# sp-uhh/audio-visual-vad

Measured on AMD Instinct MI355X. Metric: AV frame-pairs/sec (fwd+bwd), higher is better.
Workload: dtype f32; 1 GPU; AV_net fused training step (WaveNet-W0 encoder + ResNet-18 trunk + concat + 2xLSTM1024 + FC, masked BCE, backward, RCCL all-reduce, fused Adam): BASELINE configs[3]/[4] per-GPU shard; per_gpu_frame_pairs=1024, global_frame_pairs=1024, sequences_per_gpu=64, parallelism=dp1, reserved_cus=0, reported_block=median

## Files before the change

audio-visual-vad_amd/csrc/wavenet.hip:

```cpp
#include "gemm_api.h"
#include "wn_block.h"
#include "wn_tail.h"

namespace {

static inline int grid1(long n) { long b = (n + 255) / 256; return (int)(b > 8192 ? 8192 : (b < 1 ? 1 : b)); }

__global__ void conv1d_fwd_generic(const float* __restrict__ x, const float* __restrict__ w, const float* __restrict__ bias,
                                   const float* __restrict__ res, float* __restrict__ y, int B, int Cin, int Cout, int Lin,
                                   int Lout, int fw, int dil, int relu_in, int res_off, int res_L) {
  const long n = (long)B * Cout * Lout;
  for (long i = (long)blockIdx.x * blockDim.x + threadIdx.x; i < n; i += (long)gridDim.x * blockDim.x) {
    const int t = (int)(i % Lout);
    const int co = (int)((i / Lout) % Cout);
    const int b = (int)(i / ((long)Lout * Cout));
    float acc = bias ? bias[co] : 0.f;
    const float* xb = x + (long)b * Cin * Lin + t;
    const float* wr = w + (long)co * Cin * fw;
    for (int ci = 0; ci < Cin; ++ci)
      for (int k = 0; k < fw; ++k) {
        float v = xb[(long)ci * Lin + k * dil];
        if (relu_in) v = fmaxf(v, 0.f);
        acc = fmaf(wr[ci * fw + k], v, acc);
      }
    if (res) acc += res[((long)b * Cout + co) * res_L + t + res_off];
    y[i] = acc;
  }
}

__global__ void conv1d_bwd_data_generic(const float* __restrict__ dy, const float* __restrict__ w,
                                        const float* __restrict__ xmask, const float* __restrict__ res, float* __restrict__ dx,
                                        int B, int Cin, int Cout, int Lin, int Lout, int fw, int dil, int res_off, int res_L) {
  const long n = (long)B * Cin * Lin;
  for (long i = (long)blockIdx.x * blockDim.x + threadIdx.x; i < n; i += (long)gridDim.x * blockDim.x) {
    const int ti = (int)(i % Lin);
    const int ci = (int)((i / Lin) % Cin);
    const int b = (int)(i / ((long)Lin * Cin));
    float acc = 0.f;
    if (!xmask || xmask[i] > 0.f) {
      for (int k = 0; k < fw; ++k) {
        const int to = ti - k * dil;
        if (to < 0 || to >= Lout) continue;
        const float* dyb = dy + (long)b * Cout * Lout + to;
        for (int co = 0; co < Cout; ++co) acc = fmaf(w[((long)co * Cin + ci) * fw + k], dyb[(long)co * Lout], acc);
      }
    }
    if (res && ti >= res_off && ti - res_off < res_L) acc += res[((long)b * Cin + ci) * res_L + ti - res_off];
    dx[i] = acc;
  }
}

__global__ void __launch_bounds__(256) chan_sum_acc(const float* __restrict__ dy, float* __restrict__ db, int B, int C, int L) {
  __shared__ float sm[256];
  const int c = blockIdx.x;
  float s = 0.f;
  for (int b = blockIdx.y; b < B; b += gridDim.y) {
    const float* p = dy + ((long)b * C + c) * L;
    for (int t = threadIdx.x; t < L; t += 256) s += p[t];
  }
  sm[threadIdx.x] = s;
  __syncthreads();
  for (int o = 128; o > 0; o >>= 1) {
    if (threadIdx.x < o) sm[threadIdx.x] += sm[threadIdx.x + o];
    __syncthreads();
  }
  if (threadIdx.x == 0) db[c] += sm[0];
}

__global__ void __launch_bounds__(256)
    narrow_conv1d_grads(const float* __restrict__ dy, const float* __restrict__ x, float* __restrict__ part,
                        int B, int Cout, int Cin, int Lout, int Lin, int fw) {
  __shared__ float sm[5][256];
  const int co = blockIdx.x, nw = Cin * fw;
  float acc[5] = {0.f, 0.f, 0.f, 0.f, 0.f};
  for (int b = blockIdx.y; b < B; b += gridDim.y) {
    const float* p = dy + ((long)b * Cout + co) * Lout;
    const float* xb = x + (long)b * Cin * Lin;
    for (int t = threadIdx.x; t < Lout; t += 256) {
      const float g = p[t];
      acc[4] += g;
#pragma unroll
      for (int j = 0; j < 4; ++j)
        if (j < nw) acc[j] = fmaf(g, xb[(long)(j / fw) * Lin + t + (j % fw)], acc[j]);
    }
  }
#pragma unroll
  for (int j = 0; j < 5; ++j) sm[j][threadIdx.x] = acc[j];
  __syncthreads();
  for (int o = 128; o > 0; o >>= 1) {
    if (threadIdx.x < o)
#pragma unroll
      for (int j = 0; j < 5; ++j) sm[j][threadIdx.x] += sm[j][threadIdx.x + o];
    __syncthreads();
  }
  if (threadIdx.x < 5) part[((long)blockIdx.y * Cout + co) * 5 + threadIdx.x] = sm[threadIdx.x][0];
}
__global__ void narrow_conv1d_grads_sum(const float* __restrict__ part, int ny, int Cout, int nw, float* __restrict__ dw,
                                        float* __restrict__ db) {
  const int i = blockIdx.x * blockDim.x + threadIdx.x;
  if (i >= Cout * 5) return;
  const int co = i / 5, j = i - co * 5;
  float s = 0.f;
  for (int y = 0; y < ny; ++y) s += part[((long)y * Cout + co) * 5 + j];
  if (j < 4) { if (j < nw && dw) dw[(long)co * nw + j] += s; }
  else if (db) db[co] += s;
}

template <int MODE>
__global__ void __launch_bounds__(256)
    wn_block_fwd_mfma(const float* __restrict__ s_in, const float* __restrict__ w_dil, const float* __restrict__ b_dil,
                      const float* __restrict__ w_dense, const float* __restrict__ b_dense, float* __restrict__ s_out,
                      float* __restrict__ z_out, int B, int Lin, int dil) {
  static_assert(MODE == 0 || MODE == 2, "s_out only, or z only");
  const int lane = threadIdx.x & 63;
  const int li = lane & 31, lh = lane >> 5;
  const int Lo = Lin - dil;
  const int tiles_per_seq = tiles_per_sequence<32>(Lo);
  const long ntiles = (long)B * tiles_per_seq;
  const long wave0 = ((long)blockIdx.x * blockDim.x + threadIdx.x) >> 6;
  const long nwaves = ((long)gridDim.x * blockDim.x) >> 6;

  __shared__ float wl[WIMG_SIZE];
  stage_block_weights(wl, w_dil, b_dil, w_dense, b_dense, threadIdx.x, 256);
  __syncthreads();
  float wd[32];
#pragma unroll
  for (int s = 0; s < 32; ++s) wd[s] = wl[WIMG_DIL + li * WIMG_DIL_PITCH + s * 2 + lh];
  float we[16];
#pragma unroll
  for (int r = 0; r < 16; ++r) we[r] = wl[WIMG_DENSE + li * WIMG_DENSE_PITCH + mfma32_row(r, lh)];
  const float* bzl = wl + WIMG_BDIL;
  const float* bsl = wl + WIMG_BDENSE;

  float xn[32], rn[16];
  auto issue = [&](long tile) {
    const TilePos p = tile_pos(tile < ntiles ? tile : ntiles - 1, tiles_per_seq, li, Lo);
    const int b = p.b, tcl = p.ok ? p.t : 0;
    const float* xp = s_in + (long)b * 32 * Lin + tcl + lh * dil;
#pragma unroll
    for (int c = 0; c < 32; ++c) xn[c] = xp[(long)c * Lin];
    if (MODE == 0) {
      const float* rp = s_in + (long)b * 32 * Lin + tcl + dil;
#pragma unroll
      for (int r = 0; r < 16; ++r) rn[r] = rp[(long)mfma32_row(r, lh) * Lin];
    }
  };
  if (wave0 < ntiles) issue(wave0);
  for (long tile = wave0; tile < ntiles; tile += nwaves) {
    const TilePos p = tile_pos(tile, tiles_per_seq, li, Lo);
    const int b = p.b, t = p.t;
    const bool ok = p.ok;
    float x[32], rv[16];
#pragma unroll
    for (int c = 0; c < 32; ++c) x[c] = ok ? xn[c] : 0.f;
#pragma unroll
    for (int r = 0; r < 16; ++r) rv[r] = (MODE == 0 && ok) ? rn[r] : 0.f;
    issue(tile + nwaves);
    f32x16 acc;
#pragma unroll
    for (int r = 0; r < 16; ++r) acc[r] = bzl[mfma32_row(r, lh)];
#pragma unroll
    for (int s = 0; s < 32; ++s) acc = mfma32(wd[s], relu1(x[s]), acc);
    if (MODE == 2) {
      float* zp = z_out + (long)b * 32 * Lo + t;
#pragma unroll
      for (int r = 0; r < 16; ++r)
        if (ok) zp[(long)mfma32_row(r, lh) * Lo] = acc[r];
    }
    if (MODE == 0) {
      f32x16 acc2;
#pragma unroll
      for (int r = 0; r < 16; ++r) acc2[r] = bsl[mfma32_row(r, lh)] + rv[r];
#pragma unroll
      for (int r = 0; r < 16; ++r) acc2 = mfma32(we[r], relu1(acc[r]), acc2);
      float* op = s_out + (long)b * 32 * Lo + t;
#pragma unroll
      for (int r = 0; r < 16; ++r)
        if (ok) op[(long)mfma32_row(r, lh) * Lo] = acc2[r];
    }
  }
}

struct FwdTile { float x[32], r[16]; };
template <bool RESIDENT>
__device__ __forceinline__ void wn_block_fwd_body(float* wl, const float* __restrict__ s_in, const float* __restrict__ w_dil,
                                                  const float* __restrict__ b_dil, const float* __restrict__ w_dense,
                                                  const float* __restrict__ b_dense, float* __restrict__ s_out, int B, int Lin,
                                                  int dil) {
  const int lane = threadIdx.x & 63;
  const int li = lane & 31, lh = lane >> 5;
  const int Lo = Lin - dil;
  const int tiles_per_seq = tiles_per_sequence<32>(Lo);
  const int ntiles = B * tiles_per_seq;
  const float* wdl = wl + WIMG_DIL + li * WIMG_DIL_PITCH + lh;
  const float* wel = wl + WIMG_DENSE + li * WIMG_DENSE_PITCH + 4 * lh;
  const float* bzl = wl + WIMG_BDIL + 4 * lh;
  const float* bsl = wl + WIMG_BDENSE + 4 * lh;
  const int rowL = Lin * 4, rowO = Lo * 4;
  float wd[32], we[16];

  auto issue = [&](int tile, FwdTile& n) __attribute__((always_inline)) {
    const TilePos p = tile_pos(RESIDENT && tile >= ntiles ? ntiles - 1 : tile, tiles_per_seq, li, Lo);
    const __amdgpu_buffer_rsrc_t rx = brsrc(s_in + (long)p.b * 32 * Lin, 32 * rowL);
    const int offx = p.ok ? (p.t + lh * dil) * 4 : BUF_OOB;
#pragma unroll
    for (int c = 0; c < 32; ++c) n.x[c] = bload(rx, offx, c * rowL);
    const int offr = p.ok ? (p.t + dil) * 4 + 4 * lh * rowL : BUF_OOB;
#pragma unroll
    for (int r = 0; r < 16; ++r) n.r[r] = bload(rx, offr, mfma32_row(r, 0) * rowL);
  };
  auto compute = [&](int tile, const FwdTile& c) __attribute__((always_inline)) {
    const TilePos p = tile_pos(tile, tiles_per_seq, li, Lo);
    const int offo = p.ok ? p.t * 4 + 4 * lh * rowO : BUF_OOB;
    f32x16 acc;
#pragma unroll
    for (int r = 0; r < 16; ++r) acc[r] = bzl[mfma32_row(r, 0)];
#pragma unroll
    for (int s = 0; s < 32; ++s) acc = mfma32(RESIDENT ? wd[s] : wdl[2 * s], relu1(c.x[s]), acc);
    f32x16 acc2;
#pragma unroll
    for (int r = 0; r < 16; ++r) acc2[r] = bsl[mfma32_row(r, 0)] + c.r[r];
#pragma unroll
    for (int r = 0; r < 16; ++r) acc2 = mfma32(RESIDENT ? we[r] : wel[mfma32_row(r, 0)], relu1(acc[r]), acc2);
    const __amdgpu_buffer_rsrc_t ro = brsrc(s_out + (long)p.b * 32 * Lo, 32 * rowO);
#pragma unroll
    for (int r = 0; r < 16; ++r) bstore(acc2[r], ro, offo, mfma32_row(r, 0) * rowO);
  };
  const TileWalkI w = xcd_walk_i(ntiles);
  FwdTile ta, tb;
  if (RESIDENT && w.first < w.last) issue(w.first, ta);
  stage_block_weights(wl, w_dil, b_dil, w_dense, b_dense, threadIdx.x, 256);
  __syncthreads();
  if (RESIDENT) {
#pragma unroll
    for (int s = 0; s < 32; ++s) wd[s] = wdl[2 * s];
#pragma unroll
    for (int r = 0; r < 16; ++r) we[r] = wel[mfma32_row(r, 0)];
    pingpong_tiles<false>(w, ta, tb, issue, compute);
  } else {
    plain_tiles<false, FwdTile>(w, issue, compute);
  }
}

__global__ void __launch_bounds__(256)
    wn_block_fwd_buf(const float* __restrict__ s_in, const float* __restrict__ w_dil, const float* __restrict__ b_dil,
                     const float* __restrict__ w_dense, const float* __restrict__ b_dense, float* __restrict__ s_out, int B,
                     int Lin, int dil) {
  __shared__ float wl[WIMG_SIZE];
  wn_block_fwd_body<true>(wl, s_in, w_dil, b_dil, w_dense, b_dense, s_out, B, Lin, dil);
}

__global__ void __launch_bounds__(256, 4)
    wn_block_fwd_occ(const float* __restrict__ s_in, const float* __restrict__ w_dil, const float* __restrict__ b_dil,
                     const float* __restrict__ w_dense, const float* __restrict__ b_dense, float* __restrict__ s_out, int B,
                     int Lin, int dil) {
  __shared__ float wl[WIMG_SIZE];
  wn_block_fwd_body<false>(wl, s_in, w_dil, b_dil, w_dense, b_dense, s_out, B, Lin, dil);
}

__global__ void __launch_bounds__(512, 4)
    wn_block_fwd_dma(const float* __restrict__ s_in, const float* __restrict__ w_dil, const float* __restrict__ b_dil,
                     const float* __restrict__ w_dense, const float* __restrict__ b_dense, float* __restrict__ s_out, int B, int Lin,
                     int dil) {
  const int lane = threadIdx.x & 63, wave = threadIdx.x >> 6;
  const int li = lane & 31, lh = lane >> 5;
  const int Lo = Lin - dil;
  const int tiles_per_seq = tiles_per_sequence<32>(Lo);
  const int ntiles = B * tiles_per_seq;
  __shared__ __attribute__((aligned(16))) float wl[8 * 2048 + WIMG_SIZE];
  float* const wts = wl + 8 * 2048;
  stage_block_weights(wts, w_dil, b_dil, w_dense, b_dense, threadIdx.x, 512);
  __syncthreads();
  const float* wdl = wts + WIMG_DIL + li * WIMG_DIL_PITCH + lh;
  const float* wel = wts + WIMG_DENSE + li * WIMG_DENSE_PITCH + 4 * lh;
  const float* bzl = wts + WIMG_BDIL + 4 * lh;
  const float* bsl = wts + WIMG_BDENSE + 4 * lh;
  const int rowL = Lin * 4, rowO = Lo * 4;
  float* const tb = wl + __builtin_amdgcn_readfirstlane(wave) * 2048;
  const float* const xs = tb + lh * 1024 + li;
  const float* const rs = tb + 1024 + 4 * lh * 32 + li;
  const int dvo = (lane >> 3) * rowL + (lane & 7) * 16;
  const TileWalkI w = xcd_walk_i(ntiles, 8);
  for (int tile = w.first; tile < w.last; tile += w.stride) {
    const TilePos p = tile_pos(tile, tiles_per_seq, li, Lo);
    const int b = p.b, t0 = p.t0;
    const __amdgpu_buffer_rsrc_t rx = brsrc(s_in + (long)b * 32 * Lin, 32 * rowL);
#pragma unroll
    for (int q = 0; q < 4; ++q)
      __builtin_amdgcn_raw_ptr_buffer_load_lds(rx, (__attribute__((address_space(3))) void*)(tb + q * 256), 16, dvo + t0 * 4,
                                               8 * q * rowL, 0, 0);
#pragma unroll
    for (int q = 0; q < 4; ++q)
      __builtin_amdgcn_raw_ptr_buffer_load_lds(rx, (__attribute__((address_space(3))) void*)(tb + 1024 + q * 256), 16,
                                               dvo + (t0 + dil) * 4, 8 * q * rowL, 0, 0);
    const int offo = p.ok ? p.t * 4 + 4 * lh * rowO : BUF_OOB;
    f32x16 acc;
#pragma unroll
    for (int r = 0; r < 16; ++r) acc[r] = bzl[mfma32_row(r, 0)];
    asm volatile("s_waitcnt vmcnt(0)" ::: "memory");
    __builtin_amdgcn_sched_barrier(0);
    float wv[2][8], xv[2][8];
#pragma unroll
    for (int k = 0; k < 8; ++k) { wv[0][k] = wdl[2 * k]; xv[0][k] = xs[32 * k]; }
#pragma unroll
    for (int gq = 0; gq < 4; ++gq) {
      if (gq < 3) {
#pragma unroll
        for (int k = 0; k < 8; ++k) { wv[(gq + 1) & 1][k] = wdl[2 * (8 * (gq + 1) + k)]; xv[(gq + 1) & 1][k] = xs[32 * (8 * (gq + 1) + k)]; }
      }
      __builtin_amdgcn_sched_barrier(0);
#pragma unroll
      for (int k = 0; k < 8; ++k) acc = mfma32(wv[gq & 1][k], relu1(xv[gq & 1][k]), acc);
    }
    float we16[16];
    f32x16 acc2;
#pragma unroll
    for (int r = 0; r < 16; ++r) { we16[r] = wel[mfma32_row(r, 0)]; acc2[r] = bsl[mfma32_row(r, 0)] + rs[32 * mfma32_row(r, 0)]; }
    __builtin_amdgcn_sched_barrier(0);
#pragma unroll
    for (int r = 0; r < 16; ++r) acc2 = mfma32(we16[r], relu1(acc[r]), acc2);
    const __amdgpu_buffer_rsrc_t ro = brsrc(s_out + (long)b * 32 * Lo, 32 * rowO);
#pragma unroll
    for (int r = 0; r < 16; ++r) bstore(acc2[r], ro, offo, mfma32_row(r, 0) * rowO);
    __builtin_amdgcn_sched_barrier(0);
  }
}

__global__ void __launch_bounds__(256, 2)
    wn_block_fwd_w4(const float* __restrict__ s_in, const float* __restrict__ w_dil, const float* __restrict__ b_dil,
                    const float* __restrict__ w_dense, const float* __restrict__ b_dense, float* __restrict__ s_out, int B,
                    int Lin, int dil) {
  const int lane = threadIdx.x & 63;
  const int li = lane & 31, lh = lane >> 5;
  const int Lo = Lin - dil;
  const int tiles_per_seq = tiles_per_sequence<128>(Lo);
  const int ntiles = B * tiles_per_seq;
  __shared__ float wl[WIMG_SIZE];
  stage_block_weights(wl, w_dil, b_dil, w_dense, b_dense, threadIdx.x, 256);
  __syncthreads();
  const float* wdl = wl + WIMG_DIL + li * WIMG_DIL_PITCH + lh;
  const float* wel = wl + WIMG_DENSE + li * WIMG_DENSE_PITCH + 4 * lh;
  const float* bzl = wl + WIMG_BDIL + 4 * lh;
  const float* bsl = wl + WIMG_BDENSE + 4 * lh;
  const int rowL = Lin * 4, rowO = Lo * 4;

  const TileWalkI w = xcd_walk_i(ntiles);
  for (int tile = w.first; tile < w.last; tile += w.stride) {
    const TilePos p = tile_pos<128>(tile, tiles_per_seq, 4 * li, Lo);
    const int b = p.b, t0 = p.t0, t = p.t;
    const __amdgpu_buffer_rsrc_t rx = brsrc(s_in + (long)b * 32 * Lin, 32 * rowL);
    const __amdgpu_buffer_rsrc_t ro = brsrc(s_out + (long)b * 32 * Lo, 32 * rowO);
    const int offx = (t + lh * dil) * 4;
    f4v x[32];
#pragma unroll
    for (int c = 0; c < 32; ++c) x[c] = bload4(rx, offx, c * rowL);
    __builtin_amdgcn_sched_barrier(0);
    const float* wd_t = wdl;
    const float* we_t = wel;
    asm volatile("" : "+v"(wd_t), "+v"(we_t));
    f32x16 acc[4];
#pragma unroll
    for (int j = 0; j < 4; ++j)
#pragma unroll
      for (int r = 0; r < 16; ++r) acc[j][r] = bzl[mfma32_row(r, 0)];
#pragma unroll
    for (int s = 0; s < 32; ++s) {
      const float w = wd_t[2 * s];
#pragma unroll
      for (int j = 0; j < 4; ++j) acc[j] = mfma32(w, relu1(x[s][j]), acc[j]);
    }
    const int offr = (t + dil) * 4 + 4 * lh * rowL;
    f4v rv[16];
#pragma unroll
    for (int r = 0; r < 16; ++r) rv[r] = bload4(rx, offr, mfma32_row(r, 0) * rowL);
    __builtin_amdgcn_sched_barrier(0);
    f32x16 acc2[4];
#pragma unroll
    for (int j = 0; j < 4; ++j)
#pragma unroll
      for (int r = 0; r < 16; ++r) acc2[j][r] = bsl[mfma32_row(r, 0)];
#pragma unroll
    for (int r = 0; r < 16; ++r) {
      const float w = we_t[mfma32_row(r, 0)];
#pragma unroll
      for (int j = 0; j < 4; ++j) acc2[j] = mfma32(w, relu1(acc[j][r]), acc2[j]);
    }
    const int offo = t * 4 + 4 * lh * rowO;
    if (t0 + 128 <= Lo) {
#pragma unroll
      for (int r = 0; r < 16; ++r) {
        const f4v o = {acc2[0][r] + rv[r][0], acc2[1][r] + rv[r][1], acc2[2][r] + rv[r][2], acc2[3][r] + rv[r][3]};
        rv[r] = o;
      }
      __builtin_amdgcn_sched_barrier(0);
#pragma unroll
      for (int r = 0; r < 16; ++r) bstore4(rv[r], ro, offo, mfma32_row(r, 0) * rowO);
      __builtin_amdgcn_sched_barrier(0);
      asm volatile("s_nop 1");
    } else {
#pragma unroll
      for (int j = 0; j < 4; ++j) {
        const int oj = t + j < Lo ? offo + 4 * j : BUF_OOB;
#pragma unroll
        for (int r = 0; r < 16; ++r) bstore(acc2[j][r] + rv[r][j], ro, oj, mfma32_row(r, 0) * rowO);
      }
    }
  }
}


__global__ void __launch_bounds__(256)
    wn_block_bwd_dz_mfma(const float* __restrict__ dS, const float* __restrict__ Z, const float* __restrict__ w_dense,
                         float* __restrict__ DZ, int B, int Lo) {
  const int lane = threadIdx.x & 63;
  const int li = lane & 31, lh = lane >> 5;
  const int tiles_per_seq = tiles_per_sequence<32>(Lo);
  const long ntiles = (long)B * tiles_per_seq;
  const long wave0 = ((long)blockIdx.x * blockDim.x + threadIdx.x) >> 6;
  const long nwaves = ((long)gridDim.x * blockDim.x) >> 6;
  __shared__ float wl[WIMG_DENSE_SIZE];
  stage_w_dense(wl, w_dense, threadIdx.x, 256);
  __syncthreads();
  float wt[16];
#pragma unroll
  for (int s = 0; s < 16; ++s) wt[s] = wl[(2 * s + lh) * WIMG_DENSE_PITCH + li];
  for (long tile = wave0; tile < ntiles; tile += nwaves) {
    const TilePos p = tile_pos(tile, tiles_per_seq, li, Lo);
    const int b = p.b, t = p.t;
    const bool ok = p.ok;
    const long base = (long)b * 32 * Lo + (ok ? t : 0);
    float g[16], z[16];
#pragma unroll
    for (int s = 0; s < 16; ++s) g[s] = dS[base + (long)(2 * s + lh) * Lo];
#pragma unroll
    for (int r = 0; r < 16; ++r) z[r] = Z[base + (long)mfma32_row(r, lh) * Lo];
#pragma unroll
    for (int s = 0; s < 16; ++s) g[s] = ok ? g[s] : 0.f;
    f32x16 acc;
#pragma unroll
    for (int r = 0; r < 16; ++r) acc[r] = 0.f;
#pragma unroll
    for (int s = 0; s < 16; ++s) acc = mfma32(wt[s], g[s], acc);
#pragma unroll
    for (int r = 0; r < 16; ++r)
      if (ok) DZ[base + (long)mfma32_row(r, lh) * Lo] = z[r] > 0.f ? acc[r] : 0.f;
  }
}

__global__ void __launch_bounds__(256)
    wn_block_bwd_dx_mfma(const float* __restrict__ DZ, const float* __restrict__ s_in, const float* __restrict__ dS_out,
                         const float* __restrict__ w_dil, float* __restrict__ dS_in, int B, int Lin, int dil) {
  const int lane = threadIdx.x & 63;
  const int li = lane & 31, lh = lane >> 5;
  const int Lo = Lin - dil;
  const int tiles_per_seq = tiles_per_sequence<32>(Lin);
  const long ntiles = (long)B * tiles_per_seq;
  __shared__ float wl[WIMG_DIL_SIZE];
  stage_w_dil(wl, w_dil, threadIdx.x, 256);
  __syncthreads();
  float wt[32];
#pragma unroll
  for (int s = 0; s < 32; ++s) wt[s] = wl[s * WIMG_DIL_PITCH + li * 2 + lh];
  float dzn[32], svn[16], rvn[16];
  auto issue = [&](long tile) {
    const TilePos p = tile_pos(tile < ntiles ? tile : ntiles - 1, tiles_per_seq, li, Lin);
    const int b = p.b, t = p.t;
    const bool ok = p.ok;
    const int to = t - lh * dil;
    const bool okz = ok && to >= 0 && to < Lo;
    const float* zp = DZ + (long)b * 32 * Lo + (okz ? to : 0);
#pragma unroll
    for (int s = 0; s < 32; ++s) dzn[s] = zp[(long)s * Lo];
    const bool okr = ok && t >= dil;
    const float* sp = s_in + (long)b * 32 * Lin + (ok ? t : 0);
    const float* rp = dS_out + (long)b * 32 * Lo + (okr ? t - dil : 0);
#pragma unroll
    for (int r = 0; r < 16; ++r) { svn[r] = sp[(long)mfma32_row(r, lh) * Lin]; rvn[r] = rp[(long)mfma32_row(r, lh) * Lo]; }
  };
  const TileWalk tw = xcd_walk(ntiles);
  if (tw.first < tw.last) issue(tw.first);
  for (long tile = tw.first; tile < tw.last; tile += tw.stride) {
    const TilePos p = tile_pos(tile, tiles_per_seq, li, Lin);
    const int b = p.b, t = p.t;
    const bool ok = p.ok;
    const int to = t - lh * dil;
    const bool okz = ok && to >= 0 && to < Lo;
    const bool okr = ok && t >= dil;
    float dz[32], sv[16], rv[16];
#pragma unroll
    for (int s = 0; s < 32; ++s) dz[s] = okz ? dzn[s] : 0.f;
#pragma unroll
    for (int r = 0; r < 16; ++r) { sv[r] = svn[r]; rv[r] = okr ? rvn[r] : 0.f; }
    issue(tile + tw.stride);
    f32x16 acc;
#pragma unroll
    for (int r = 0; r < 16; ++r) acc[r] = 0.f;
#pragma unroll
    for (int s = 0; s < 32; ++s) acc = mfma32(wt[s], dz[s], acc);
    float* op = dS_in + (long)b * 32 * Lin + t;
#pragma unroll
    for (int r = 0; r < 16; ++r)
      if (ok) op[(long)mfma32_row(r, lh) * Lin] = (sv[r] > 0.f ? acc[r] : 0.f) + rv[r];
  }
}

struct DxTile { float dz[32], sv[16], rv[16]; };
template <bool RESIDENT>
__device__ __forceinline__ void wn_block_bwd_dx_body(float* wl, const float* __restrict__ DZ, const float* __restrict__ s_in,
                                                     const float* __restrict__ dS_out, const float* __restrict__ w_dil,
                                                     float* __restrict__ dS_in, int B, int Lin, int dil) {
  const int lane = threadIdx.x & 63;
  const int li = lane & 31, lh = lane >> 5;
  const int Lo = Lin - dil;
  const int tiles_per_seq = tiles_per_sequence<32>(Lin);
  const int ntiles = B * tiles_per_seq;
  const float* wtl = wl + li * 2 + lh;
  const int rowL = Lin * 4, rowO = Lo * 4;
  float wt[32];
  auto issue = [&](int tile, DxTile& n) __attribute__((always_inline)) {
    const TilePos p = tile_pos(RESIDENT && tile >= ntiles ? ntiles - 1 : tile, tiles_per_seq, li, Lin);
    const int t = p.t;
    const int to = t - lh * dil;
    const bool okz = p.ok && to >= 0 && to < Lo;
    const bool okr = p.ok && t >= dil;
    const __amdgpu_buffer_rsrc_t rz = brsrc(DZ + (long)p.b * 32 * Lo, 32 * rowO);
    const __amdgpu_buffer_rsrc_t rs = brsrc(s_in + (long)p.b * 32 * Lin, 32 * rowL);
    const __amdgpu_buffer_rsrc_t rg = brsrc(dS_out + (long)p.b * 32 * Lo, 32 * rowO);
    const int offz = okz ? to * 4 : BUF_OOB;
    const int offs = p.ok ? t * 4 + 4 * lh * rowL : BUF_OOB;
    const int offg = okr ? (t - dil) * 4 + 4 * lh * rowO : BUF_OOB;
#pragma unroll
    for (int s = 0; s < 32; ++s) n.dz[s] = bload(rz, offz, s * rowO);
#pragma unroll
    for (int r = 0; r < 16; ++r) { n.sv[r] = bload(rs, offs, mfma32_row(r, 0) * rowL); n.rv[r] = bload(rg, offg, mfma32_row(r, 0) * rowO); }
  };
  auto compute = [&](int tile, const DxTile& c) __attribute__((always_inline)) {
    const TilePos p = tile_pos(tile, tiles_per_seq, li, Lin);
    const __amdgpu_buffer_rsrc_t ro = brsrc(dS_in + (long)p.b * 32 * Lin, 32 * rowL);
    const int offs = p.ok ? p.t * 4 + 4 * lh * rowL : BUF_OOB;
    f32x16 acc;
#pragma unroll
    for (int r = 0; r < 16; ++r) acc[r] = 0.f;
#pragma unroll
    for (int s = 0; s < 32; ++s) acc = mfma32(RESIDENT ? wt[s] : wtl[WIMG_DIL_PITCH * s], c.dz[s], acc);
#pragma unroll
    for (int r = 0; r < 16; ++r) bstore((c.sv[r] > 0.f ? acc[r] : 0.f) + c.rv[r], ro, offs, mfma32_row(r, 0) * rowL);
  };
  const TileWalkI w = xcd_walk_i(ntiles);
  DxTile ta, tb;
  if (RESIDENT && w.first < w.last) issue(w.first, ta);
  stage_w_dil(wl, w_dil, threadIdx.x, 256);
  __syncthreads();
  if (RESIDENT) {
#pragma unroll
    for (int s = 0; s < 32; ++s) wt[s] = wtl[WIMG_DIL_PITCH * s];
    pingpong_tiles<false>(w, ta, tb, issue, compute);
  } else {
    plain_tiles<false, DxTile>(w, issue, compute);
  }
}

__global__ void __launch_bounds__(256)
    wn_block_bwd_dx_buf(const float* __restrict__ DZ, const float* __restrict__ s_in, const float* __restrict__ dS_out,
                        const float* __restrict__ w_dil, float* __restrict__ dS_in, int B, int Lin, int dil) {
  __shared__ float wl[WIMG_DIL_SIZE];
  wn_block_bwd_dx_body<true>(wl, DZ, s_in, dS_out, w_dil, dS_in, B, Lin, dil);
}

__global__ void __launch_bounds__(256, 4)
    wn_block_bwd_dx_occ(const float* __restrict__ DZ, const float* __restrict__ s_in, const float* __restrict__ dS_out,
                        const float* __restrict__ w_dil, float* __restrict__ dS_in, int B, int Lin, int dil) {
  __shared__ float wl[WIMG_DIL_SIZE];
  wn_block_bwd_dx_body<false>(wl, DZ, s_in, dS_out, w_dil, dS_in, B, Lin, dil);
}

constexpr int WG_SLAB = 3 * 1024 + 64;
constexpr int WG_MAXBLK = 512;

__global__ void __launch_bounds__(256)
    wn_block_wgrad_mfma(const float* __restrict__ dS, const float* __restrict__ Z, const float* __restrict__ DZ,
                        const float* __restrict__ s_in, float* __restrict__ slab, int B, int Lin, int dil) {
  __shared__ float tile[4][32 * 33];
  __shared__ float red[WG_SLAB];
  const int lane = threadIdx.x & 63, wave = threadIdx.x >> 6;
  const int li = lane & 31, lh = lane >> 5;
  const int Lo = Lin - dil;
  const int tiles_per_seq = tiles_per_sequence<32>(Lo);
  const long ntiles = (long)B * tiles_per_seq;
  const long wave0 = ((long)blockIdx.x * blockDim.x + threadIdx.x) >> 6;
  const long nwaves = ((long)gridDim.x * blockDim.x) >> 6;
  float* T = tile[wave];
  for (int i = threadIdx.x; i < WG_SLAB; i += 256) red[i] = 0.f;

  f32x16 acc0, acc1, acc2;
#pragma unroll
  for (int r = 0; r < 16; ++r) { acc0[r] = 0.f; acc1[r] = 0.f; acc2[r] = 0.f; }
  float bs_dz = 0.f, bs_ds = 0.f;

  auto gl = [&](const float* base, long rstride, float (&v)[16]) {
#pragma unroll
    for (int q = 0; q < 16; ++q) v[q] = base[(long)(2 * q + lh) * rstride];
  };
  auto xpose = [&](const float (&v)[16], bool ok, bool relu, float (&f)[16]) {
    __builtin_amdgcn_wave_barrier();
#pragma unroll
    for (int q = 0; q < 16; ++q) {
      const float x = ok ? v[q] : 0.f;
      T[(2 * q + lh) * 33 + li] = relu ? relu1(x) : x;
    }
    __builtin_amdgcn_wave_barrier();
#pragma unroll
    for (int q = 0; q < 16; ++q) f[q] = T[li * 33 + 2 * q + lh];
    __builtin_amdgcn_wave_barrier();
  };

  for (long tl = wave0; tl < ntiles; tl += nwaves) {
    const TilePos p = tile_pos(tl, tiles_per_seq, li, Lo);
    const int b = p.b, t = p.t;
    const bool ok = p.ok;
    const long oo = (long)b * 32 * Lo + (ok ? t : 0);
    const long oi = (long)b * 32 * Lin + (ok ? t : 0);
    float v0[16], v1[16], v2[16], v3[16], v4[16];
    gl(DZ + oo, Lo, v0);
    gl(s_in + oi, Lin, v1);
    gl(s_in + oi + dil, Lin, v2);
    gl(dS + oo, Lo, v3);
    gl(Z + oo, Lo, v4);
    float fa[16], fb[16];
    xpose(v0, ok, false, fa);
#pragma unroll
    for (int q = 0; q < 16; ++q) bs_dz += fa[q];
    xpose(v1, ok, true, fb);
#pragma unroll
    for (int q = 0; q < 16; ++q) acc0 = mfma32(fa[q], fb[q], acc0);
    xpose(v2, ok, true, fb);
#pragma unroll
    for (int q = 0; q < 16; ++q) acc1 = mfma32(fa[q], fb[q], acc1);
    xpose(v3, ok, false, fa);
#pragma unroll
    for (int q = 0; q < 16; ++q) bs_ds += fa[q];
    xpose(v4, ok, true, fb);
#pragma unroll
    for (int q = 0; q < 16; ++q) acc2 = mfma32(fa[q], fb[q], acc2);
  }

  __syncthreads();
#pragma unroll
  for (int r = 0; r < 16; ++r) {
    const int row = mfma32_row(r, lh);
    atomicAdd(&red[row * 32 + li], acc0[r]);
    atomicAdd(&red[1024 + row * 32 + li], acc1[r]);
    atomicAdd(&red[2048 + row * 32 + li], acc2[r]);
  }
  atomicAdd(&red[3072 + li], bs_dz);
  atomicAdd(&red[3104 + li], bs_ds);
  __syncthreads();
  float* out = slab + (long)blockIdx.x * WG_SLAB;
  for (int i = threadIdx.x; i < WG_SLAB; i += 256) out[i] = red[i];
}

struct DzwTile { float g[16], x[32]; };
template <bool RESIDENT>
__device__ __forceinline__ void wn_block_bwd_dz_wgrad_body(float* tiles, float* red, float* wl, float* wtl,
                                                           const float* __restrict__ dS, const float* __restrict__ w_dil,
                                                           const float* __restrict__ b_dil, const float* __restrict__ w_dense,
                                                           const float* __restrict__ s_in, float* __restrict__ DZ,
                                                           float* __restrict__ slab, int B, int Lin, int dil) {
  const int lane = threadIdx.x & 63, wave = threadIdx.x >> 6;
  const int li = lane & 31, lh = lane >> 5;
  const int Lo = Lin - dil;
  const int tiles_per_seq = tiles_per_sequence<32>(Lo);
  const int ntiles = B * tiles_per_seq;
  float* T = tiles + wave * 2 * 1056;
  float* T1 = T + 1056;
  float* Th = T + lh * 1056;
  stage_w_dil(wl, w_dil, threadIdx.x, 256);
  stage_bias(wl + WIMG_DIL_SIZE, b_dil, threadIdx.x);
  if (RESIDENT) stage_w_dense(T, w_dense, lane, 64);
  else stage_w_dense(wtl, w_dense, threadIdx.x, 256);
  for (int i = threadIdx.x; i < WG_SLAB; i += 256) red[i] = 0.f;
  __syncthreads();
  const float* wtp = (RESIDENT ? T : wtl) + lh * WIMG_DENSE_PITCH + li;
  const float* wdp = wl + li * WIMG_DIL_PITCH + lh;
  const float* bzl = wl + WIMG_DIL_SIZE + 4 * lh;
  float wt[16], wd[32];
  if (RESIDENT) {
#pragma unroll
    for (int s = 0; s < 16; ++s) wt[s] = wtp[2 * WIMG_DENSE_PITCH * s];
#pragma unroll
    for (int s = 0; s < 32; ++s) wd[s] = wdp[2 * s];
  }
  __builtin_amdgcn_wave_barrier();

  f32x16 acc0, acc1, acc2;
#pragma unroll
  for (int r = 0; r < 16; ++r) { acc0[r] = 0.f; acc1[r] = 0.f; acc2[r] = 0.f; }
  float bs_dz = 0.f, bs_ds = 0.f;
  const int rowL = Lin * 4, rowO = Lo * 4;

  auto issue = [&](int tile, DzwTile& n) __attribute__((always_inline)) {
    const TilePos p = tile_pos(tile < ntiles ? tile : ntiles - 1, tiles_per_seq, li, Lo);
    const __amdgpu_buffer_rsrc_t rg = brsrc(dS + (long)p.b * 32 * Lo, 32 * rowO);
    const __amdgpu_buffer_rsrc_t rx = brsrc(s_in + (long)p.b * 32 * Lin, 32 * rowL);
    const int offg = p.ok ? p.t * 4 + lh * rowO : BUF_OOB;
    const int offx = p.ok ? (p.t + lh * dil) * 4 : BUF_OOB;
#pragma unroll
    for (int q = 0; q < 16; ++q) n.g[q] = bload(rg, offg, 2 * q * rowO);
#pragma unroll
    for (int c = 0; c < 32; ++c) n.x[c] = bload(rx, offx, c * rowL);
  };
  auto compute = [&](int tidx, const DzwTile& c) __attribute__((always_inline)) {
    const TilePos p = tile_pos(tidx, tiles_per_seq, li, Lo);
    const int offo = p.ok ? p.t * 4 + 4 * lh * rowO : BUF_OOB;
    const __amdgpu_buffer_rsrc_t rz = brsrc(DZ + (long)p.b * 32 * Lo, 32 * rowO);
    float x[32];
#pragma unroll
    for (int s = 0; s < 32; ++s) x[s] = relu1(c.x[s]);
    f32x16 z;
#pragma unroll
    for (int r = 0; r < 16; ++r) z[r] = bzl[mfma32_row(r, 0)];
#pragma unroll
    for (int s = 0; s < 32; ++s) z = mfma32(RESIDENT ? wd[s] : wdp[2 * s], x[s], z);
    f32x16 acc;
#pragma unroll
    for (int r = 0; r < 16; ++r) acc[r] = 0.f;
#pragma unroll
    for (int q = 0; q < 16; ++q) acc = mfma32(RESIDENT ? wt[q] : wtp[2 * WIMG_DENSE_PITCH * q], c.g[q], acc);
    float f0[16], f1[16];
    __builtin_amdgcn_wave_barrier();
#pragma unroll
    for (int r = 0; r < 16; ++r) {
      const float dz = z[r] > 0.f ? acc[r] : 0.f;
      bstore(dz, rz, offo, mfma32_row(r, 0) * rowO);
      T[mfma32_row(r, lh) * 33 + li] = dz;
    }
    __builtin_amdgcn_wave_barrier();
#pragma unroll
    for (int q = 0; q < 16; ++q) { f0[q] = T[li * 33 + 2 * q + lh]; bs_dz += f0[q]; }
    __builtin_amdgcn_wave_barrier();
#pragma unroll
    for (int s = 0; s < 32; ++s) Th[s * 33 + li] = x[s];
    __builtin_amdgcn_wave_barrier();
#pragma unroll
    for (int q = 0; q < 16; ++q) f1[q] = T[li * 33 + 2 * q + lh];
#pragma unroll
    for (int q = 0; q < 16; ++q) acc0 = mfma32(f0[q], f1[q], acc0);
#pragma unroll
    for (int q = 0; q < 16; ++q) f1[q] = T1[li * 33 + 2 * q + lh];
#pragma unroll
    for (int q = 0; q < 16; ++q) acc1 = mfma32(f0[q], f1[q], acc1);
    __builtin_amdgcn_wave_barrier();
#pragma unroll
    for (int q = 0; q < 16; ++q) T[(2 * q + lh) * 33 + li] = c.g[q];
#pragma unroll
    for (int r = 0; r < 16; ++r) T1[mfma32_row(r, lh) * 33 + li] = relu1(z[r]);
    __builtin_amdgcn_wave_barrier();
#pragma unroll
    for (int q = 0; q < 16; ++q) { f0[q] = T[li * 33 + 2 * q + lh]; bs_ds += f0[q]; }
#pragma unroll
    for (int q = 0; q < 16; ++q) f1[q] = T1[li * 33 + 2 * q + lh];
#pragma unroll
    for (int q = 0; q < 16; ++q) acc2 = mfma32(f0[q], f1[q], acc2);
    __builtin_amdgcn_wave_barrier();
  };
  const TileWalkI w = xcd_walk_i(ntiles);
  DzwTile ta, tb;
  if (RESIDENT) {
    if (w.first < w.last) issue(w.first, ta);
    pingpong_tiles<true>(w, ta, tb, issue, compute);
  } else {
    plain_tiles<true, DzwTile>(w, issue, compute);
  }

  for (int wv = 0; wv < 4; ++wv) {
    __syncthreads();
    if (wave == wv) {
#pragma unroll
      for (int r = 0; r < 16; ++r) {
        const int row = mfma32_row(r, lh);
        red[row * 32 + li] += acc0[r];
        red[1024 + row * 32 + li] += acc1[r];
        red[2048 + row * 32 + li] += acc2[r];
      }
      if (lh == 0) { red[3072 + li] += bs_dz; red[3104 + li] += bs_ds; }
      __builtin_amdgcn_wave_barrier();
      if (lh == 1) { red[3072 + li] += bs_dz; red[3104 + li] += bs_ds; }
    }
  }
  __syncthreads();
  float* out = slab + (long)blockIdx.x * WG_SLAB;
  for (int i = threadIdx.x; i < WG_SLAB; i += 256) out[i] = red[i];
}

__global__ void __launch_bounds__(256)
    wn_block_bwd_dz_wgrad_mfma(const float* __restrict__ dS, const float* __restrict__ w_dil, const float* __restrict__ b_dil,
                               const float* __restrict__ w_dense, const float* __restrict__ s_in, float* __restrict__ DZ,
                               float* __restrict__ slab, int B, int Lin, int dil) {
  __shared__ float tile[4 * 2 * 32 * 33];
  __shared__ float red[WG_SLAB];
  __shared__ float wl[WIMG_DIL_SIZE + 32];
  wn_block_bwd_dz_wgrad_body<true>(tile, red, wl, nullptr, dS, w_dil, b_dil, w_dense, s_in, DZ, slab, B, Lin, dil);
}

__global__ void __launch_bounds__(256, 2)
    wn_block_bwd_dz_wgrad_occ(const float* __restrict__ dS, const float* __restrict__ w_dil, const float* __restrict__ b_dil,
                               const float* __restrict__ w_dense, const float* __restrict__ s_in, float* __restrict__ DZ,
                               float* __restrict__ slab, int B, int Lin, int dil) {
  __shared__ float tile[4 * 2 * 32 * 33];
  __shared__ float red[WG_SLAB];
  __shared__ float wl[WIMG_DIL_SIZE + 32];
  __shared__ float wtl[WIMG_DENSE_SIZE];
  wn_block_bwd_dz_wgrad_body<false>(tile, red, wl, wtl, dS, w_dil, b_dil, w_dense, s_in, DZ, slab, B, Lin, dil);
}

typedef float f4u __attribute__((ext_vector_type(4), aligned(4)));

__global__ void __launch_bounds__(256, 2)
    wn_block_bwd_dzw_t(const float* __restrict__ dS, const float* __restrict__ w_dil, const float* __restrict__ b_dil,
                       const float* __restrict__ w_dense, const float* __restrict__ s_in, float* __restrict__ DZ,
                       float* __restrict__ slab, int B, int Lin, int dil) {
  __shared__ float red[WG_SLAB];
  __shared__ float wl[WIMG_BDENSE];
  const int lane = threadIdx.x & 63;
  const int li = lane & 31, lh = lane >> 5;
  const int Lo = Lin - dil;
  const int tiles_per_seq = tiles_per_sequence<32>(Lo);
  const long ntiles = (long)B * tiles_per_seq;
  const long wave0 = ((long)blockIdx.x * blockDim.x + threadIdx.x) >> 6;
  const long nwaves = ((long)gridDim.x * blockDim.x) >> 6;
  stage_w_dil(wl + WIMG_DIL, w_dil, threadIdx.x, 256);
  stage_w_dense(wl + WIMG_DENSE, w_dense, threadIdx.x, 256);
  stage_bias(wl + WIMG_BDIL, b_dil, threadIdx.x);
  for (int i = threadIdx.x; i < WG_SLAB; i += 256) red[i] = 0.f;
  __syncthreads();
  const float* wdp = wl + WIMG_DIL + li * WIMG_DIL_PITCH + lh;
  const float* wtp = wl + WIMG_DENSE + lh * WIMG_DENSE_PITCH + li;
  const float bz = wl[WIMG_BDIL + li];

  f32x16 acc0, acc1, acc2;
#pragma unroll
  for (int r = 0; r < 16; ++r) { acc0[r] = 0.f; acc1[r] = 0.f; acc2[r] = 0.f; }
  float bs_dz = 0.f, bs_ds = 0.f;

  for (long tl = wave0; tl < ntiles; tl += nwaves) {
    const TilePos p = tile_pos(tl, tiles_per_seq, li, Lo);
    const int b = p.b, t0 = p.t0, t = p.t;
    const bool ok = p.ok;
    const int tcl = ok ? t : 0;
    const bool full = t0 + 32 <= Lo;
    float x[32], g[16];
    {
      const float* xp = s_in + (long)b * 32 * Lin + tcl + lh * dil;
#pragma unroll
      for (int c = 0; c < 32; ++c) x[c] = xp[(long)c * Lin];
      const float* gp = dS + (long)b * 32 * Lo + tcl;
#pragma unroll
      for (int q = 0; q < 16; ++q) g[q] = gp[(long)(2 * q + lh) * Lo];
    }
    float gc[16], xc0[16], xc1[16];
    const float* rowS = dS + ((long)b * 32 + li) * Lo + t0 + 4 * lh;
    const float* rowX = s_in + ((long)b * 32 + li) * Lin + t0 + 4 * lh;
    if (full) {
#pragma unroll
      for (int q = 0; q < 4; ++q) {
        const f4u a = *reinterpret_cast<const f4u*>(rowS + 8 * q);
        const f4u u = *reinterpret_cast<const f4u*>(rowX + 8 * q);
        const f4u v = *reinterpret_cast<const f4u*>(rowX + dil + 8 * q);
#pragma unroll
        for (int e = 0; e < 4; ++e) { gc[4 * q + e] = a[e]; xc0[4 * q + e] = u[e]; xc1[4 * q + e] = v[e]; }
      }
    } else {
#pragma unroll
      for (int s = 0; s < 16; ++s) {
        const int o = 8 * (s >> 2) + (s & 3);
        const bool in = t0 + 4 * lh + o < Lo;
        const int oc = in ? o : -(t0 + 4 * lh);
        const float a = rowS[oc], u = rowX[oc], v = rowX[oc + dil];
        gc[s] = in ? a : 0.f; xc0[s] = in ? u : 0.f; xc1[s] = in ? v : 0.f;
      }
    }
    __builtin_amdgcn_sched_barrier(0);
#pragma unroll
    for (int c = 0; c < 32; ++c) x[c] = ok ? relu1(x[c]) : 0.f;
#pragma unroll
    for (int q = 0; q < 16; ++q) g[q] = ok ? g[q] : 0.f;
    f32x16 zT;
#pragma unroll
    for (int r = 0; r < 16; ++r) zT[r] = bz;
#pragma unroll
    for (int s = 0; s < 32; ++s) zT = mfma32(x[s], wdp[2 * s], zT);
    f32x16 dzT;
#pragma unroll
    for (int r = 0; r < 16; ++r) dzT[r] = 0.f;
#pragma unroll
    for (int s = 0; s < 16; ++s) dzT = mfma32(g[s], wtp[66 * s], dzT);
#pragma unroll
    for (int r = 0; r < 16; ++r) dzT[r] = zT[r] > 0.f ? dzT[r] : 0.f;
    float* rowZ = DZ + ((long)b * 32 + li) * Lo + t0 + 4 * lh;
    if (full) {
#pragma unroll
      for (int q = 0; q < 4; ++q) {
        f4u o = {dzT[4 * q], dzT[4 * q + 1], dzT[4 * q + 2], dzT[4 * q + 3]};
        *reinterpret_cast<f4u*>(rowZ + 8 * q) = o;
      }
    } else {
#pragma unroll
      for (int s = 0; s < 16; ++s) {
        const int o = 8 * (s >> 2) + (s & 3);
        if (t0 + 4 * lh + o < Lo) rowZ[o] = dzT[s];
      }
    }
#pragma unroll
    for (int s = 0; s < 16; ++s) { bs_dz += dzT[s]; bs_ds += gc[s]; }
#pragma unroll
    for (int s = 0; s < 16; ++s) acc2 = mfma32(gc[s], relu1(zT[s]), acc2);
#pragma unroll
    for (int s = 0; s < 16; ++s) acc0 = mfma32(dzT[s], relu1(xc0[s]), acc0);
#pragma unroll
    for (int s = 0; s < 16; ++s) acc1 = mfma32(dzT[s], relu1(xc1[s]), acc1);
  }

#pragma unroll
  for (int r = 0; r < 16; ++r) {
    const int row = mfma32_row(r, lh);
    atomicAdd(&red[row * 32 + li], acc0[r]);
    atomicAdd(&red[1024 + row * 32 + li], acc1[r]);
    atomicAdd(&red[2048 + row * 32 + li], acc2[r]);
  }
  atomicAdd(&red[3072 + li], bs_dz);
  atomicAdd(&red[3104 + li], bs_ds);
  __syncthreads();
  float* out = slab + (long)blockIdx.x * WG_SLAB;
  for (int i = threadIdx.x; i < WG_SLAB; i += 256) out[i] = red[i];
}

constexpr int WN_MAXL = 64;
struct WgradTab {
  const float* slab[WN_MAXL];
  int nslab[WN_MAXL];
  float* dW_dil[WN_MAXL];
  float* db_dil[WN_MAXL];
  float* dW_dense[WN_MAXL];
  float* db_dense[WN_MAXL];
};
__global__ void __launch_bounds__(256) wn_wgrad_reduce_all(const WgradTab tab) {
  const int l = blockIdx.y;
  const int i = blockIdx.x * 32 + (threadIdx.x & 31);
  const int nslab = tab.nslab[l];
  const float s = slab_sum_fixed_order(tab.slab[l] + i, nslab, WG_SLAB);
  if (threadIdx.x >= 32 || nslab <= 0) return;
  if (i < 2048) { if (tab.dW_dil[l]) tab.dW_dil[l][(i & 1023) * 2 + (i >> 10)] += s; }
  else if (i < 3072) { if (tab.dW_dense[l]) tab.dW_dense[l][i - 2048] += s; }
  else if (i < 3104) { if (tab.db_dil[l]) tab.db_dil[l][i - 3072] += s; }
  else if (tab.db_dense[l]) tab.db_dense[l][i - 3104] += s;
}

struct Plan {
  int n;
  int L[66];
  size_t s[66];
  size_t z, dz, ga, gb, dzt;
  size_t zs[66];
  size_t slab;
  size_t gslab;
  size_t total;
};
static int make_plan(const avvad_wavenet_desc* d, Plan* p) {
  if (!d || d->n_layers < 0 || d->n_layers > 64 || d->B <= 0 || d->fw < 1 || d->qc < 1 || d->R < 1 || d->D < 1 ||
      d->Bn < 1 || d->P < 1 || (d->n_layers > 0 && !d->dilations_h))
    return AVVAD_EINVAL;
  p->n = d->n_layers;
  p->L[0] = d->L - (d->fw - 1);
  for (int i = 0; i < p->n; ++i) p->L[i + 1] = p->L[i] - d->dilations_h[i] * (d->fw - 1);
  if (p->L[p->n] < 1) return AVVAD_EINVAL;
  size_t off = 0;
  auto take = [&](size_t n) { size_t o = off; off += align_up(n, 64); return o; };
  const size_t B = d->B;
  if (d->save_for_backward) {
    for (int i = 0; i <= p->n; ++i) p->s[i] = take(B * d->R * p->L[i]);
    const size_t big = B * (size_t)(d->R > d->D ? d->R : d->D) * p->L[0];
    p->z = take(big); p->dz = take(big); p->ga = take(big); p->gb = take(big);
    p->dzt = take(B * d->Bn * p->L[p->n]);
    {
      const size_t zb = (d->R == 32 && d->D == 32 && d->fw == 2 && p->n > 0) ? take(B * d->D * p->L[1]) : 0;
      for (int i = 0; i < p->n; ++i) p->zs[i] = zb;
    }
    {
      const bool perlayer = d->R == 32 && d->D == 32 && d->fw == 2;
      const size_t a = (size_t)WG_MAXBLK * WG_SLAB * (perlayer ? (size_t)p->n : 1), b2 = (size_t)TAIL_MAXBLK * tail_slab_floats(d->Bn);
      p->slab = take(a > b2 ? a : b2);
    }
    p->gslab = take(igemm::SLAB_FLOATS);
  } else {
    for (int i = 0; i < p->n; ++i) p->zs[i] = 0;
    const size_t a = take(B * d->R * p->L[0]), b2 = take(B * d->R * p->L[0]);
    for (int i = 0; i <= p->n; ++i) p->s[i] = (i & 1) ? b2 : a;
    p->z = take(B * d->D * p->L[0]);
    p->dz = p->ga = p->gb = p->dzt = 0;
  }
  p->total = off;
  return AVVAD_OK;
}

static inline bool mfma_shape(const avvad_wavenet_desc* d) { return d->R == 32 && d->D == 32 && d->fw == 2; }
static inline bool buf_ok(int B, int Lin) {
  return avvad_tune().wn_flat != 1 && (long)Lin * 32 * 4 + 4096 < (1L << 31) && (long)B * cdiv(Lin, 32) < (1L << 31);
}

enum class FwdForm { FLAT, BUF, OCC, WIDE, DMA };
enum class DxForm { FLAT, BUF, OCC };
enum class BwdForm { RESIDENT, OCC, TRANSPOSED, UNFUSED };
enum class TailFwdForm { GENERIC, MFMA1, MFMA4 };
enum class TailBwdForm { PAIR, FUSED, MFMA, GENERIC };
struct FwdChoice { FwdForm form; int grid; };
struct DxChoice { DxForm form; int grid; };
struct BwdChoice { BwdForm form; int grid; int grid_z, grid_dz; };
struct TailFwdChoice { TailFwdForm form; int grid; };
struct TailBwdChoice { TailBwdForm form; int grid; };

enum class XcdRound { NONE, UP, UP_FROM_8, DOWN_FROM_8 };
static int wn_grid_size(long tiles, int per_wg, long cap, int wn_grid, XcdRound r) {
  long g = (tiles + per_wg - 1) / per_wg;
  if (g > cap) g = cap;
  if (wn_grid > 0 && g > wn_grid) g = wn_grid;
  if (r == XcdRound::UP || (r == XcdRound::UP_FROM_8 && g >= 8)) g = (g + 7) / 8 * 8;
  if (r == XcdRound::DOWN_FROM_8 && g >= 8) g = g / 8 * 8;
  return (int)(g < 1 ? 1 : g);
}

constexpr int WIDE_FROM = 8192;
static FwdChoice fwd_form(int B, int Lin, int dil) {
  const AvvadTune& t = avvad_tune();
  const int Lo = Lin - dil;
  const bool buf = buf_ok(B, Lin);
  if (buf && (t.wn_flat == 0 || t.wn_flat == 3) && Lo >= 128 && (Lo >= WIDE_FROM || t.wn_flat == 3))
    return {FwdForm::WIDE, wn_grid_size((long)B * cdiv(Lo, 128), 4, t.wn_grid > 0 ? t.wn_grid : 1024, 0, XcdRound::UP)};
  const long ntiles = (long)B * cdiv(Lo, 32);
  if (buf && t.wn_flat == 5 && Lo >= 32)
    return {FwdForm::DMA, wn_grid_size(ntiles, 8, 512, t.wn_grid, XcdRound::UP_FROM_8)};
  if (buf && (t.wn_flat == 0 || t.wn_flat == 4))
    return {FwdForm::OCC, wn_grid_size(ntiles, 4, 1024, t.wn_grid, XcdRound::UP_FROM_8)};
  return {buf ? FwdForm::BUF : FwdForm::FLAT, wn_grid_size(ntiles, 4, 512, t.wn_grid, XcdRound::NONE)};
}

static DxChoice dx_form(int B, int Lin) {
  const AvvadTune& t = avvad_tune();
  const long ntiles = (long)B * cdiv(Lin, 32);
  if (buf_ok(B, Lin) && (t.wn_dx == 0 || t.wn_dx == 2))
    return {DxForm::OCC, wn_grid_size(ntiles, 4, 1024, 0, XcdRound::UP_FROM_8)};
  return {buf_ok(B, Lin) && t.wn_dx != 3 ? DxForm::BUF : DxForm::FLAT, wn_grid_size(ntiles, 4, 512, 0, XcdRound::NONE)};
}

static BwdChoice bwd_form(int B, int Lo, bool shared_device, bool any_grad) {
  const AvvadTune& t = avvad_tune();
  const long ntiles = (long)B * cdiv(Lo, 32);
  if (!any_grad || t.wn_no_fused_wgrad)
    return {BwdForm::UNFUSED, wn_grid_size(ntiles, 16, WG_MAXBLK, 0, XcdRound::NONE), wn_grid_size(ntiles, 4, 512, 0, XcdRound::NONE),
            wn_grid_size(ntiles, 4, 768, 0, XcdRound::NONE)};
  switch (t.wn_bwd_t == 0 ? (shared_device ? 3 : 2) : t.wn_bwd_t) {
    case 3:
      return {BwdForm::RESIDENT, wn_grid_size(ntiles, 16, 256, 0, XcdRound::NONE), 0, 0};
    case 2:
      return {BwdForm::OCC, wn_grid_size(ntiles, 16, WG_MAXBLK, 0, XcdRound::DOWN_FROM_8), 0, 0};
    default:
      return {BwdForm::TRANSPOSED, wn_grid_size(ntiles, 16, WG_MAXBLK, 0, XcdRound::NONE), 0, 0};
  }
}

static TailFwdChoice tail_fwd_form(int B, int R, int Bn, int P) {
  if (!(R == 32 && Bn % 32 == 0)) return {TailFwdForm::GENERIC, 0};
  const int nt = Bn % 128 == 0 ? 4 : 1;
  return {nt == 4 ? TailFwdForm::MFMA4 : TailFwdForm::MFMA1, wn_grid_size((long)B * P * (Bn / (32 * nt)), 4, 2048, 0, XcdRound::NONE)};
}

static TailBwdChoice tail_bwd_form(int B, int Lv, int R, int Bn, int P, bool any_grad) {
  const AvvadTune& t = avvad_tune();
  const long ntiles = (long)B * cdiv(Lv, 32);
  if (!(R == 32 && Bn % 32 == 0 && Bn <= 1024) || P > Lv) return {TailBwdForm::GENERIC, 0};
  if (Bn == 256 && any_grad && !t.wn_no_fused_tail)
    return {t.wn_no_tail_pair ? TailBwdForm::FUSED : TailBwdForm::PAIR, wn_grid_size(ntiles, 4, TAIL_MAXBLK, 0, XcdRound::NONE)};
  return {TailBwdForm::MFMA, wn_grid_size(ntiles, 4, 2048, 0, XcdRound::NONE)};
}

static void launch_block_fwd(const float* s_in, const float* wd, const float* bd, const float* we, const float* be, float* s_out,
                             int B, int Lin, int dil, hipStream_t s) {
  const FwdChoice c = fwd_form(B, Lin, dil);
  const dim3 grid(c.grid);
  switch (c.form) {
    case FwdForm::WIDE: hipLaunchKernelGGL(wn_block_fwd_w4, grid, dim3(256), 0, s, s_in, wd, bd, we, be, s_out, B, Lin, dil); break;
    case FwdForm::DMA: hipLaunchKernelGGL(wn_block_fwd_dma, grid, dim3(512), 0, s, s_in, wd, bd, we, be, s_out, B, Lin, dil); break;
    case FwdForm::OCC: hipLaunchKernelGGL(wn_block_fwd_occ, grid, dim3(256), 0, s, s_in, wd, bd, we, be, s_out, B, Lin, dil); break;
    case FwdForm::BUF: hipLaunchKernelGGL(wn_block_fwd_buf, grid, dim3(256), 0, s, s_in, wd, bd, we, be, s_out, B, Lin, dil); break;
    case FwdForm::FLAT:
      hipLaunchKernelGGL(wn_block_fwd_mfma<0>, grid, dim3(256), 0, s, s_in, wd, bd, we, be, s_out, (float*)nullptr, B, Lin, dil);
      break;
  }
}

static int wgrad_conv1d(const float* dy, const float* x, float* dw, int B, int Cout, int Cin, int Lout, int Lin, int fw,
                        int dil, int relu_in, hipStream_t s, float* slab) {
  const long K = (long)B * Lout;
  if (K > 0x7fffffffL) return AVVAD_EINVAL;
  const int ktiles = cdiv(K, igemm::BK);
  int split = 1024 / (cdiv(Cout, 64) * cdiv(Cin * fw, 64));
  if (split > ktiles) split = ktiles;
  if (split < 1) split = 1;
  igemm::RowSegK a{dy, Lout, (long)Cout * Lout, Cout, (int)K, Lout, 0, 0, 1, 0};
  igemm::RowSegK b{x, Lin, (long)Cin * Lin, Cin * fw, (int)K, Lout, 0, relu_in, fw, dil};
  igemm::EpiStore e{dw, (long)Cin * fw, nullptr, 1};
  return igemm::launch<64, 64>(a, b, e, Cout, Cin * fw, (int)K, split, s, slab);
}

static void bias_grad(const float* dy, float* db, int B, int C, int L, hipStream_t s) {
  if (!db) return;
  hipLaunchKernelGGL(chan_sum_acc, dim3(C, 1), dim3(256), 0, s, dy, db, B, C, L);
}

static void launch_tail_fwd(const float* sN, const float* wb, const float* bb, float* out, int B, int R, int Bn, int Lv, int P,
                            hipStream_t s) {
  const TailFwdChoice c = tail_fwd_form(B, R, Bn, P);
  switch (c.form) {
    case TailFwdForm::MFMA4: hipLaunchKernelGGL(tail_fwd_mfma<4>, dim3(c.grid), dim3(256), 0, s, sN, wb, bb, out, B, Bn, Lv, P); break;
    case TailFwdForm::MFMA1: hipLaunchKernelGGL(tail_fwd_mfma<1>, dim3(c.grid), dim3(256), 0, s, sN, wb, bb, out, B, Bn, Lv, P); break;
    case TailFwdForm::GENERIC: hipLaunchKernelGGL(tail_fwd_generic, dim3(P, B), dim3(256), 0, s, sN, wb, bb, out, R, Bn, Lv, P); break;
  }
}

static int launch_tail_bwd(const float* sN, const float* wb, const float* bb, const float* dout, float* dW, float* db, float* dS,
                           float* dzt, float* slab, float* gslab, int B, int R, int Bn, int Lv, int P, hipStream_t s) {
  const TailBwdChoice c = tail_bwd_form(B, Lv, R, Bn, P, dW || db);
  int rc;
  if (c.form == TailBwdForm::PAIR || c.form == TailBwdForm::FUSED) {
    const bool pair = c.form == TailBwdForm::PAIR;
    const size_t lds = (size_t)tail_fused_lds_floats(Bn, pair ? 2 : 1) * sizeof(float);
    if ((rc = pair ? allow_large_lds<tail_bwd_wgrad_pair<8>>(lds, lds) : allow_large_lds<tail_bwd_wgrad_mfma<8>>(lds, lds))) return rc;
    hipLaunchKernelGGL(pair ? tail_bwd_wgrad_pair<8> : tail_bwd_wgrad_mfma<8>, dim3(c.grid), dim3(pair ? 512 : 256), lds, s, sN, wb,
                       bb, dout, dS, slab, B, Lv, P);
    hipLaunchKernelGGL(tail_wgrad_reduce, dim3(cdiv(tail_slab_floats(Bn), 32)), dim3(256), 0, s, slab, c.grid, Bn, dW, db);
    return AVVAD_OK;
  }
  if (c.form == TailBwdForm::MFMA)
    hipLaunchKernelGGL(tail_bwd_mfma, dim3(c.grid), dim3(256), (size_t)tail_wimg_floats(Bn) * sizeof(float), s, sN, wb, bb, dout,
                       dzt, dS, B, Bn, Lv, P);
  else
    hipLaunchKernelGGL(tail_bwd_dz_generic, dim3(grid1((long)B * Bn * Lv)), dim3(256), 0, s, sN, wb, bb, dout, dzt, B, R, Bn, Lv, P);
  if (dW && (rc = wgrad_conv1d(dzt, sN, dW, B, Bn, R, Lv, Lv, 1, 1, 0, s, gslab))) return rc;
  bias_grad(dzt, db, B, Bn, Lv, s);
  if (c.form == TailBwdForm::GENERIC)
    hipLaunchKernelGGL(conv1d_bwd_data_generic, dim3(grid1((long)B * R * Lv)), dim3(256), 0, s, dzt, wb, (const float*)nullptr,
                       (const float*)nullptr, dS, B, R, Bn, Lv, Lv, 1, 1, 0, 0);
  return AVVAD_OK;
}

}

extern "C" size_t avvad_wavenet_workspace(const avvad_wavenet_desc* d) {
  Plan p;
  if (make_plan(d, &p)) return 0;
  return p.total * sizeof(float);
}

extern "C" int avvad_wavenet_fwd(const float* wave, const avvad_wavenet_params* prm, float* out, const avvad_wavenet_desc* d,
                                 void* wsv, size_t ws_bytes, avvad_stream_t sv) {
  AVVAD_ENTER();
  Plan p;
  if (!wave || !prm || !out || !wsv || ws_misaligned(wsv) || make_plan(d, &p)) return AVVAD_EINVAL;
  if (ws_bytes < p.total * sizeof(float)) return AVVAD_EWORKSPACE;
  hipStream_t s = (hipStream_t)sv;
  float* ws = (float*)wsv;
  const int B = d->B, R = d->R, D = d->D, fw = d->fw;
  hipLaunchKernelGGL(conv1d_fwd_generic, dim3(grid1((long)B * R * p.L[0])), dim3(256), 0, s, wave, prm->causal_w,
                     d->use_bias ? prm->causal_b : (const float*)nullptr, (const float*)nullptr, ws + p.s[0], B, d->qc, R,
                     d->L, p.L[0], fw, 1, 0, 0, 0);
  for (int i = 0; i < p.n; ++i) {
    const int dil = d->dilations_h[i];
    const float* bd = d->use_bias ? prm->dil_b_h[i] : nullptr;
    const float* be = d->use_bias ? prm->dense_b_h[i] : nullptr;
    if (mfma_shape(d)) {
      launch_block_fwd(ws + p.s[i], prm->dil_w_h[i], bd, prm->dense_w_h[i], be, ws + p.s[i + 1], B, p.L[i], dil, s);
    } else {
      float* z = ws + p.z;
      hipLaunchKernelGGL(conv1d_fwd_generic, dim3(grid1((long)B * D * p.L[i + 1])), dim3(256), 0, s, ws + p.s[i],
                         prm->dil_w_h[i], bd, (const float*)nullptr, z, B, R, D, p.L[i], p.L[i + 1], fw, dil, 1, 0, 0);
      hipLaunchKernelGGL(conv1d_fwd_generic, dim3(grid1((long)B * R * p.L[i + 1])), dim3(256), 0, s, z, prm->dense_w_h[i], be,
                         ws + p.s[i], ws + p.s[i + 1], B, D, R, p.L[i + 1], p.L[i + 1], 1, 1, 1, p.L[i] - p.L[i + 1], p.L[i]);
    }
  }
  launch_tail_fwd(ws + p.s[p.n], prm->bott_w, d->use_bias ? prm->bott_b : (const float*)nullptr, out, B, R, d->Bn, p.L[p.n],
                  d->P, s);
  AVVAD_LAUNCH_CHECK();
  return AVVAD_OK;
}

extern "C" int avvad_wavenet_block_fwd(const float* s_in, const float* w_dil, const float* b_dil, const float* w_dense,
                                       const float* b_dense, float* s_out, int B, int Lin, int dil, avvad_stream_t sv) {
  AVVAD_ENTER();
  if (!s_in || !w_dil || !w_dense || !s_out || B <= 0 || dil < 1 || Lin - dil < 1) return AVVAD_EINVAL;
  launch_block_fwd(s_in, w_dil, b_dil, w_dense, b_dense, s_out, B, Lin, dil, (hipStream_t)sv);
  AVVAD_LAUNCH_CHECK();
  return AVVAD_OK;
}

extern "C" int avvad_wavenet_bwd(const float* wave, const avvad_wavenet_params* prm, const float* dout,
                                 const avvad_wavenet_grads* g, float* dwave, const avvad_wavenet_desc* d, void* wsv,
                                 size_t ws_bytes, avvad_stream_t sv) {
  AVVAD_ENTER();
  Plan p;
  if (!wave || !prm || !dout || !g || !wsv || ws_misaligned(wsv) || make_plan(d, &p) || !d->save_for_backward) return AVVAD_EINVAL;
  if (ws_bytes < p.total * sizeof(float)) return AVVAD_EWORKSPACE;
  hipStream_t s = (hipStream_t)sv;
  float* ws = (float*)wsv;
  const int B = d->B, R = d->R, D = d->D, fw = d->fw, Bn = d->Bn;
  int rc;
  float* Z = ws + p.z;
  float* DZ = ws + p.dz;
  float* GA = ws + p.ga;
  float* GB = ws + p.gb;
  if ((rc = launch_tail_bwd(ws + p.s[p.n], prm->bott_w, d->use_bias ? prm->bott_b : (const float*)nullptr, dout, g->bott_w,
                            d->use_bias ? g->bott_b : (float*)nullptr, GA, ws + p.dzt, ws + p.slab, ws + p.gslab, B, R, Bn,
                            p.L[p.n], d->P, s)))
    return rc;
  WgradTab wtab;
  bool any_slab = false;
  for (int l = 0; l < WN_MAXL; ++l) {
    wtab.slab[l] = nullptr; wtab.nslab[l] = 0;
    wtab.dW_dil[l] = wtab.db_dil[l] = wtab.dW_dense[l] = wtab.db_dense[l] = nullptr;
  }
  auto note_slabs = [&](int i, float* slab_i, int wb) {
    wtab.slab[i] = slab_i; wtab.nslab[i] = wb;
    wtab.dW_dil[i] = g->dil_w_h[i]; wtab.dW_dense[i] = g->dense_w_h[i];
    wtab.db_dil[i] = d->use_bias ? g->dil_b_h[i] : (float*)nullptr;
    wtab.db_dense[i] = d->use_bias ? g->dense_b_h[i] : (float*)nullptr;
    any_slab = true;
  };
  for (int i = p.n - 1; i >= 0; --i) {
    float* const slab_i = ws + p.slab + (size_t)i * WG_MAXBLK * WG_SLAB;
    const int dil = d->dilations_h[i];
    const int Li = p.L[i], Lo = p.L[i + 1];
    const float* si = ws + p.s[i];
    const float* bd = d->use_bias ? prm->dil_b_h[i] : nullptr;
    const bool fast = mfma_shape(d);
    float* Zi = fast ? ws + p.zs[i] : Z;
    if (!fast)
      hipLaunchKernelGGL(conv1d_fwd_generic, dim3(grid1((long)B * D * Lo)), dim3(256), 0, s, si, prm->dil_w_h[i], bd,
                         (const float*)nullptr, Zi, B, R, D, Li, Lo, fw, dil, 1, 0, 0);
    if (fast) {
      const bool any_grad = g->dil_w_h[i] || g->dense_w_h[i] || (d->use_bias && (g->dil_b_h[i] || g->dense_b_h[i]));
      const BwdChoice bc = bwd_form(B, Lo, d->shared_device != 0, any_grad);
      switch (bc.form) {
        case BwdForm::RESIDENT:
          hipLaunchKernelGGL(wn_block_bwd_dz_wgrad_mfma, dim3(bc.grid), dim3(256), 0, s, GA, prm->dil_w_h[i], bd,
                             prm->dense_w_h[i], si, DZ, slab_i, B, Li, dil);
          break;
        case BwdForm::OCC:
          hipLaunchKernelGGL(wn_block_bwd_dz_wgrad_occ, dim3(bc.grid), dim3(256), 0, s, GA, prm->dil_w_h[i], bd,
                             prm->dense_w_h[i], si, DZ, slab_i, B, Li, dil);
          break;
        case BwdForm::TRANSPOSED:
          hipLaunchKernelGGL(wn_block_bwd_dzw_t, dim3(bc.grid), dim3(256), 0, s, GA, prm->dil_w_h[i], bd, prm->dense_w_h[i], si,
                             DZ, slab_i, B, Li, dil);
          break;
        case BwdForm::UNFUSED:
          hipLaunchKernelGGL(wn_block_fwd_mfma<2>, dim3(bc.grid_z), dim3(256), 0, s, si, prm->dil_w_h[i], bd, prm->dense_w_h[i],
                             (const float*)nullptr, (float*)nullptr, Zi, B, Li, dil);
          hipLaunchKernelGGL(wn_block_bwd_dz_mfma, dim3(bc.grid_dz), dim3(256), 0, s, GA, Zi, prm->dense_w_h[i], DZ, B, Lo);
          if (any_grad)
            hipLaunchKernelGGL(wn_block_wgrad_mfma, dim3(bc.grid), dim3(256), 0, s, GA, Zi, DZ, si, slab_i, B, Li, dil);
          break;
      }
      if (any_grad) note_slabs(i, slab_i, bc.grid);
      const DxChoice dc = dx_form(B, Li);
      switch (dc.form) {
        case DxForm::OCC:
          hipLaunchKernelGGL(wn_block_bwd_dx_occ, dim3(dc.grid), dim3(256), 0, s, DZ, si, GA, prm->dil_w_h[i], GB, B, Li, dil);
          break;
        case DxForm::BUF:
          hipLaunchKernelGGL(wn_block_bwd_dx_buf, dim3(dc.grid), dim3(256), 0, s, DZ, si, GA, prm->dil_w_h[i], GB, B, Li, dil);
          break;
        case DxForm::FLAT:
          hipLaunchKernelGGL(wn_block_bwd_dx_mfma, dim3(dc.grid), dim3(256), 0, s, DZ, si, GA, prm->dil_w_h[i], GB, B, Li, dil);
          break;
      }
    } else {
      if (g->dense_w_h[i] && (rc = wgrad_conv1d(GA, Zi, g->dense_w_h[i], B, R, D, Lo, Lo, 1, 1, 1, s, ws + p.gslab))) return rc;
      if (d->use_bias) bias_grad(GA, g->dense_b_h[i], B, R, Lo, s);
      hipLaunchKernelGGL(conv1d_bwd_data_generic, dim3(grid1((long)B * D * Lo)), dim3(256), 0, s, GA, prm->dense_w_h[i], Zi,
                         (const float*)nullptr, DZ, B, D, R, Lo, Lo, 1, 1, 0, 0);
      if (g->dil_w_h[i] && (rc = wgrad_conv1d(DZ, si, g->dil_w_h[i], B, D, R, Lo, Li, fw, dil, 1, s, ws + p.gslab))) return rc;
      if (d->use_bias) bias_grad(DZ, g->dil_b_h[i], B, D, Lo, s);
      hipLaunchKernelGGL(conv1d_bwd_data_generic, dim3(grid1((long)B * R * Li)), dim3(256), 0, s, DZ, prm->dil_w_h[i], si, GA,
                         GB, B, R, D, Li, Lo, fw, dil, Li - Lo, Lo);
    }
    float* t = GA; GA = GB; GB = t;
  }
  if (any_slab) hipLaunchKernelGGL(wn_wgrad_reduce_all, dim3(WG_SLAB / 32, p.n), dim3(256), 0, s, wtab);
  if (d->qc * fw <= 4) {
    if (g->causal_w || (d->use_bias && g->causal_b))
    {
      const int ny = B < 32 ? B : 32;
      float* part = ws + p.gslab;
      hipLaunchKernelGGL(narrow_conv1d_grads, dim3(R, ny), dim3(256), 0, s, GA, wave, part, B, R, d->qc, p.L[0], d->L, fw);
      hipLaunchKernelGGL(narrow_conv1d_grads_sum, dim3(cdiv(R * 5, 256)), dim3(256), 0, s, part, ny, R, d->qc * fw, g->causal_w,
                         d->use_bias ? g->causal_b : (float*)nullptr);
    }
  } else {
    if (g->causal_w && (rc = wgrad_conv1d(GA, wave, g->causal_w, B, R, d->qc, p.L[0], d->L, fw, 1, 0, s, ws + p.gslab))) return rc;
    if (d->use_bias) bias_grad(GA, g->causal_b, B, R, p.L[0], s);
  }
  if (dwave)
    hipLaunchKernelGGL(conv1d_bwd_data_generic, dim3(grid1((long)B * d->qc * d->L)), dim3(256), 0, s, GA, prm->causal_w,
                       (const float*)nullptr, (const float*)nullptr, dwave, B, d->qc, R, d->L, p.L[0], fw, 1, 0, 0);
  AVVAD_LAUNCH_CHECK();
  return AVVAD_OK;
}
```

audio-visual-vad_amd/csrc/wn_tail.h:

```cpp
#pragma once
#include "common.h"

namespace {

constexpr int TAIL_MAXBLK = 256;
constexpr int TAIL_PITCH = 33;
constexpr int TAIL_TILE = 32 * TAIL_PITCH;
constexpr int tail_wimg_floats(int Bn) { return Bn * TAIL_PITCH; }
constexpr int tail_slab_floats(int Bn) { return Bn * 32 + Bn; }
constexpr int tail_fused_lds_floats(int Bn, int WPT) {
  return tail_wimg_floats(Bn) + tail_slab_floats(Bn) + 4 * WPT * 2 * TAIL_TILE + (WPT == 2 ? 4 * TAIL_TILE : 0);
}

__device__ __forceinline__ void pool_bin(int p, int Lv, int P, int& a, int& e) {
  a = (int)(((long)p * Lv) / P);
  e = (int)((((long)(p + 1)) * Lv + P - 1) / P);
}
__device__ __forceinline__ void stage_tail_weights(float* img, const float* __restrict__ wb, int Bn, int tid, int nthreads) {
  for (int i = tid; i < Bn * 32; i += nthreads) img[(i >> 5) * TAIL_PITCH + (i & 31)] = wb[i];
}
struct PoolWindow { int pb[3]; float pc[3]; };
__device__ __forceinline__ PoolWindow pool_window(int t, bool ok, int Lv, int P) {
  PoolWindow w;
  const int c0 = ok ? (int)(((long)t * P) / Lv) : 0;
#pragma unroll
  for (int j = 0; j < 3; ++j) {
    const int p = c0 - 1 + j;
    int a = 0, e = 0;
    const bool in = ok && p >= 0 && p < P;
    if (in) pool_bin(p, Lv, P, a, e);
    const bool hit = in && t >= a && t < e;
    w.pb[j] = hit ? p : 0;
    w.pc[j] = hit ? 1.f / (float)(e - a) : 0.f;
  }
  return w;
}
__device__ __forceinline__ f32x16 tail_z_tile(const float* wl, const float* __restrict__ bb, int nb, const float (&x)[16], int li, int lh) {
  f32x16 accZ;
#pragma unroll
  for (int r = 0; r < 16; ++r) accZ[r] = bb ? bb[nb + mfma32_row(r, lh)] : 0.f;
  float wz[16];
#pragma unroll
  for (int k = 0; k < 16; ++k) wz[k] = wl[(nb + li) * TAIL_PITCH + 2 * k + lh];
#pragma unroll
  for (int k = 0; k < 16; ++k) accZ = mfma32(wz[k], x[k], accZ);
  return accZ;
}
template <class Fetch>
__device__ __forceinline__ void tail_dz_tile(const f32x16& accZ, Fetch fetch, float (&dz)[16]) {
#pragma unroll
  for (int r = 0; r < 16; ++r) { const float g = fetch(r); dz[r] = accZ[r] > 0.f ? g : 0.f; }
}
__device__ __forceinline__ void tail_wt_frag(const float* wl, int nb, int li, int lh, float (&wt)[16]) {
#pragma unroll
  for (int k = 0; k < 16; ++k) wt[k] = wl[(nb + mfma32_row(k, lh)) * TAIL_PITCH + li];
}
__device__ __forceinline__ void tail_ds_product(f32x16& accS, const float (&wt)[16], const float (&dz)[16]) {
#pragma unroll
  for (int r = 0; r < 16; ++r) accS = mfma32(wt[r], dz[r], accS);
}
template <bool DLAYOUT>
__device__ __forceinline__ void tile_to_fragment(float* T, const float (&v)[16], float (&f)[16], int li, int lh) {
  __builtin_amdgcn_wave_barrier();
#pragma unroll
  for (int k = 0; k < 16; ++k) T[(DLAYOUT ? mfma32_row(k, lh) : 2 * k + lh) * TAIL_PITCH + li] = v[k];
  __builtin_amdgcn_wave_barrier();
#pragma unroll
  for (int q = 0; q < 16; ++q) f[q] = T[li * TAIL_PITCH + 2 * q + lh];
}
template <class Add>
__device__ __forceinline__ void meet_in_wave_order(int nwaves, int wave, Add add) {
  for (int w = 0; w < nwaves; ++w) {
    __syncthreads();
    if (wave == w) add();
  }
}
__device__ __forceinline__ float slab_sum_fixed_order(const float* __restrict__ el_ptr, int nslab, int pitch) {
  __shared__ float sm[8][32];
  const int el = threadIdx.x & 31, grp = threadIdx.x >> 5;
  float s = 0.f;
#pragma unroll 4
  for (int b = grp; b < nslab; b += 8) s += el_ptr[(long)b * pitch];
  sm[grp][el] = s;
  __syncthreads();
  if (grp == 0) {
#pragma unroll
    for (int k = 1; k < 8; ++k) s += sm[k][el];
  }
  return s;
}

__global__ void __launch_bounds__(256)
    tail_fwd_generic(const float* __restrict__ s, const float* __restrict__ wb, const float* __restrict__ bb,
                     float* __restrict__ out, int R, int Bn, int Lv, int P) {
  const int b = blockIdx.y, p = blockIdx.x;
  int a, e;
  pool_bin(p, Lv, P, a, e);
  const float* sb = s + (long)b * R * Lv;
  for (int bn = threadIdx.x; bn < Bn; bn += 256) {
    const float* wr = wb + (long)bn * R;
    const float bias = bb ? bb[bn] : 0.f;
    float sum = 0.f;
    for (int t = a; t < e; ++t) {
      float z = bias;
      for (int c = 0; c < R; ++c) z = fmaf(wr[c], sb[(long)c * Lv + t], z);
      sum += fmaxf(z, 0.f);
    }
    out[((long)b * Bn + bn) * P + p] = sum / (float)(e - a);
  }
}

__global__ void tail_bwd_dz_generic(const float* __restrict__ s, const float* __restrict__ wb, const float* __restrict__ bb,
                                    const float* __restrict__ dout, float* __restrict__ dz, int B, int R, int Bn, int Lv, int P) {
  const long n = (long)B * Bn * Lv;
  for (long i = (long)blockIdx.x * blockDim.x + threadIdx.x; i < n; i += (long)gridDim.x * blockDim.x) {
    const int t = (int)(i % Lv);
    const int bn = (int)((i / Lv) % Bn);
    const int b = (int)(i / ((long)Lv * Bn));
    float z = bb ? bb[bn] : 0.f;
    const float* sb = s + (long)b * R * Lv + t;
    for (int c = 0; c < R; ++c) z = fmaf(wb[(long)bn * R + c], sb[(long)c * Lv], z);
    float g = 0.f;
    if (z > 0.f) {
      const int p0 = (int)(((long)t * P) / Lv), p1 = (int)((((long)t + 1) * P + Lv - 1) / Lv);
      for (int p = p0; p < p1; ++p) {
        int a, e;
        pool_bin(p, Lv, P, a, e);
        g += dout[((long)b * Bn + bn) * P + p] / (float)(e - a);
      }
    }
    dz[i] = g;
  }
}

template <int NT>
__global__ void __launch_bounds__(256)
    tail_fwd_mfma(const float* __restrict__ s, const float* __restrict__ wb, const float* __restrict__ bb,
                  float* __restrict__ out, int B, int Bn, int Lv, int P) {
  const int lane = threadIdx.x & 63;
  const int li = lane & 31, lh = lane >> 5;
  const int ngrp = Bn / (32 * NT);
  const long nitems = (long)B * P * ngrp;
  const long nwaves = ((long)gridDim.x * blockDim.x) >> 6;
  for (long item = ((long)blockIdx.x * blockDim.x + threadIdx.x) >> 6; item < nitems; item += nwaves) {
    const int grp = (int)(item % ngrp);
    const int p = (int)((item / ngrp) % P);
    const int b = (int)(item / ((long)ngrp * P));
    const int bn0 = grp * 32 * NT;
    int a, e;
    pool_bin(p, Lv, P, a, e);
    float w[NT][16], bias[NT], sum[NT];
#pragma unroll
    for (int n = 0; n < NT; ++n) {
#pragma unroll
      for (int k = 0; k < 16; ++k) w[n][k] = wb[(long)(bn0 + n * 32 + li) * 32 + 2 * k + lh];
      bias[n] = bb ? bb[bn0 + n * 32 + li] : 0.f;
      sum[n] = 0.f;
    }
    const float* sp = s + (long)b * 32 * Lv;
    for (int t0 = a; t0 < e; t0 += 32) {
      const int t = t0 + li;
      const bool ok = t < e;
      const int tcl = ok ? t : a;
      float x[16];
#pragma unroll
      for (int k = 0; k < 16; ++k) x[k] = sp[(long)(2 * k + lh) * Lv + tcl];
#pragma unroll
      for (int k = 0; k < 16; ++k) x[k] = ok ? x[k] : 0.f;
#pragma unroll
      for (int n = 0; n < NT; ++n) {
        f32x16 acc = {};
#pragma unroll
        for (int k = 0; k < 16; ++k) acc = mfma32(x[k], w[n][k], acc);
#pragma unroll
        for (int r = 0; r < 16; ++r)
          if (t0 + mfma32_row(r, lh) < e) sum[n] += relu1(acc[r] + bias[n]);
      }
    }
    const float inv = 1.f / (float)(e - a);
#pragma unroll
    for (int n = 0; n < NT; ++n) {
      const float v = sum[n] + __shfl_xor(sum[n], 32, 64);
      if (lh == 0) out[((long)b * Bn + bn0 + n * 32 + li) * P + p] = v * inv;
    }
  }
}

__global__ void __launch_bounds__(256)
    tail_bwd_mfma(const float* __restrict__ s, const float* __restrict__ wb, const float* __restrict__ bb,
                  const float* __restrict__ dout, float* __restrict__ dzt, float* __restrict__ dS, int B, int Bn, int Lv, int P) {
  const int lane = threadIdx.x & 63;
  const int li = lane & 31, lh = lane >> 5;
  const int tiles_per_seq = (Lv + 31) >> 5;
  const long ntiles = (long)B * tiles_per_seq;
  const long nwaves = ((long)gridDim.x * blockDim.x) >> 6;
  extern __shared__ float wl[];
  stage_tail_weights(wl, wb, Bn, threadIdx.x, 256);
  __syncthreads();
  for (long tile = ((long)blockIdx.x * blockDim.x + threadIdx.x) >> 6; tile < ntiles; tile += nwaves) {
    const int b = (int)(tile / tiles_per_seq);
    const int t = (int)(tile - (long)b * tiles_per_seq) * 32 + li;
    const bool ok = t < Lv;
    const float* sp = s + (long)b * 32 * Lv + (ok ? t : 0);
    float x[16];
#pragma unroll
    for (int k = 0; k < 16; ++k) x[k] = sp[(long)(2 * k + lh) * Lv];
#pragma unroll
    for (int k = 0; k < 16; ++k) x[k] = ok ? x[k] : 0.f;
    const PoolWindow pw = pool_window(t, ok, Lv, P);
    f32x16 accS = {};
    for (int nb = 0; nb < Bn; nb += 32) {
      const f32x16 accZ = tail_z_tile(wl, bb, nb, x, li, lh);
      float dz[16];
      tail_dz_tile(accZ, [&](int r) {
        const long o = ((long)b * Bn + nb + mfma32_row(r, lh)) * P;
        float g = 0.f;
#pragma unroll
        for (int j = 0; j < 3; ++j) g = fmaf(dout[o + pw.pb[j]], pw.pc[j], g);
        return g;
      }, dz);
#pragma unroll
      for (int r = 0; r < 16; ++r)
        if (ok) dzt[((long)b * Bn + nb + mfma32_row(r, lh)) * Lv + t] = dz[r];
      float wt[16];
      tail_wt_frag(wl, nb, li, lh, wt);
      tail_ds_product(accS, wt, dz);
    }
#pragma unroll
    for (int r = 0; r < 16; ++r)
      if (ok) dS[((long)b * 32 + mfma32_row(r, lh)) * Lv + t] = accS[r];
  }
}

template <int NBT, int WPT>
__device__ __forceinline__ void tail_bwd_wgrad_body(const float* __restrict__ s, const float* __restrict__ wb,
                                                    const float* __restrict__ bb, const float* __restrict__ dout,
                                                    float* __restrict__ dS, float* __restrict__ slab, int B, int Lv, int P) {
  static_assert((WPT == 1 || WPT == 2) && NBT % WPT == 0, "one wave per time tile, or two that halve the bottleneck rows");
  constexpr int Bn = NBT * 32, NH = NBT / WPT, NWAVES = 4 * WPT, NTHREADS = 64 * NWAVES, SLAB = tail_slab_floats(Bn);
  extern __shared__ float wl[];
  float* red = wl + tail_wimg_floats(Bn);
  float* tiles = red + SLAB;
  const int lane = threadIdx.x & 63, wave = threadIdx.x >> 6;
  const int li = lane & 31, lh = lane >> 5;
  const int pair = wave >> 1, half = WPT == 2 ? wave & 1 : 0;
  const int tiles_per_seq = (Lv + 31) >> 5;
  const long ntiles = (long)B * tiles_per_seq;
  float *T0 = tiles + wave * 2 * TAIL_TILE, *T1 = T0 + TAIL_TILE;
  float* PS = tiles + (NWAVES * 2 + pair) * TAIL_TILE;
  stage_tail_weights(wl, wb, Bn, threadIdx.x, NTHREADS);
  for (int i = threadIdx.x; i < SLAB; i += NTHREADS) red[i] = 0.f;
  __syncthreads();
  f32x16 accW[NH] = {};
  float bsum[NH] = {};
  const int rowV = Lv * 4;
  const bool single = (Lv % P) == 0;
  auto one_tile = [&](long tile, bool live) __attribute__((always_inline)) {
    const int b = __builtin_amdgcn_readfirstlane((int)((live ? tile : 0) / tiles_per_seq));
    const int t = (int)((live ? tile : 0) - (long)b * tiles_per_seq) * 32 + li;
    const bool ok = live && t < Lv;
    const __amdgpu_buffer_rsrc_t rs = brsrc(s + (long)b * 32 * Lv, 32 * rowV);
    const __amdgpu_buffer_rsrc_t rd = brsrc(dS + (long)b * 32 * Lv, 32 * rowV);
    const __amdgpu_buffer_rsrc_t rg = brsrc(dout + (long)b * Bn * P, Bn * P * 4);
    const int offs = ok ? t * 4 + lh * rowV : BUF_OOB;
    const int offd = ok ? t * 4 + 4 * lh * rowV : BUF_OOB;
    float x[16];
#pragma unroll
    for (int k = 0; k < 16; ++k) x[k] = bload(rs, offs, 2 * k * rowV);
    __builtin_amdgcn_sched_barrier(0);
    const PoolWindow pw = pool_window(t, ok, Lv, P);
    int pbo[3];
#pragma unroll
    for (int j = 0; j < 3; ++j) pbo[j] = (pw.pb[j] + 4 * lh * P) * 4;
    float fs[16];
    tile_to_fragment<false>(T0, x, fs, li, lh);
    f32x16 accS = {};
#pragma unroll
    for (int n = 0; n < NH; ++n) {
      const int nb = (half * NH + n) * 32;
      float wt[16];
      if constexpr (WPT == 1) tail_wt_frag(wl, nb, li, lh, wt);
      const f32x16 accZ = tail_z_tile(wl, bb, nb, x, li, lh);
      if constexpr (WPT == 2) __builtin_amdgcn_sched_barrier(0);
      float dz[16];
      tail_dz_tile(accZ, [&](int r) {
        const int row = (nb + mfma32_row(r, 0)) * P * 4;
        if (single) return bload(rg, pbo[1], row) * pw.pc[1];
        float g = 0.f;
#pragma unroll
        for (int j = 0; j < 3; ++j) g = fmaf(bload(rg, pbo[j], row), pw.pc[j], g);
        return g;
      }, dz);
      if constexpr (WPT == 2) {
        __builtin_amdgcn_sched_barrier(0);
        tail_wt_frag(wl, nb, li, lh, wt);
      }
      tail_ds_product(accS, wt, dz);
      if constexpr (WPT == 2) __builtin_amdgcn_sched_barrier(0);
      float fz[16];
      tile_to_fragment<true>(T1, dz, fz, li, lh);
#pragma unroll
      for (int q = 0; q < 16; ++q) bsum[n] += fz[q];
#pragma unroll
      for (int q = 0; q < 16; ++q) accW[n] = mfma32(fz[q], fs[q], accW[n]);
    }
    if constexpr (WPT == 2) {
      if (half == 1) {
#pragma unroll
        for (int r = 0; r < 16; ++r) PS[mfma32_row(r, lh) * TAIL_PITCH + li] = accS[r];
      }
      __syncthreads();
      if (half == 0) {
#pragma unroll
        for (int r = 0; r < 16; ++r) bstore(accS[r] + PS[mfma32_row(r, lh) * TAIL_PITCH + li], rd, offd, mfma32_row(r, 0) * rowV);
      }
      __syncthreads();
    } else {
#pragma unroll
      for (int r = 0; r < 16; ++r) bstore(accS[r], rd, offd, mfma32_row(r, 0) * rowV);
    }
  };
  if constexpr (WPT == 2) {
    const long npairs = (long)gridDim.x * 4;
    const long rounds = (ntiles + npairs - 1) / npairs;
    for (long rd_ = 0; rd_ < rounds; ++rd_) {
      const long tile = rd_ * npairs + (long)blockIdx.x * 4 + pair;
      one_tile(tile, tile < ntiles);
    }
  } else {
    const long nwaves = ((long)gridDim.x * blockDim.x) >> 6;
    for (long tile = ((long)blockIdx.x * blockDim.x + threadIdx.x) >> 6; tile < ntiles; tile += nwaves) one_tile(tile, true);
  }
  meet_in_wave_order(NWAVES, wave, [&] {
#pragma unroll
    for (int n = 0; n < NH; ++n) {
#pragma unroll
      for (int r = 0; r < 16; ++r) red[((half * NH + n) * 32 + mfma32_row(r, lh)) * 32 + li] += accW[n][r];
    }
#pragma unroll
    for (int h = 0; h < 2; ++h) {
      if (h == 1) __builtin_amdgcn_wave_barrier();
#pragma unroll
      for (int n = 0; n < NH; ++n)
        if (lh == h) red[Bn * 32 + (half * NH + n) * 32 + li] += bsum[n];
    }
  });
  __syncthreads();
  float* out = slab + (long)blockIdx.x * SLAB;
  for (int i = threadIdx.x; i < SLAB; i += NTHREADS) out[i] = red[i];
}

template <int NBT>
__global__ void __launch_bounds__(256)
    tail_bwd_wgrad_mfma(const float* __restrict__ s, const float* __restrict__ wb, const float* __restrict__ bb,
                        const float* __restrict__ dout, float* __restrict__ dS, float* __restrict__ slab, int B, int Lv, int P) {
  tail_bwd_wgrad_body<NBT, 1>(s, wb, bb, dout, dS, slab, B, Lv, P);
}

template <int NBT>
__global__ void __launch_bounds__(512, 2)
    tail_bwd_wgrad_pair(const float* __restrict__ s, const float* __restrict__ wb, const float* __restrict__ bb,
                        const float* __restrict__ dout, float* __restrict__ dS, float* __restrict__ slab, int B, int Lv, int P) {
  tail_bwd_wgrad_body<NBT, 2>(s, wb, bb, dout, dS, slab, B, Lv, P);
}

__global__ void __launch_bounds__(256)
    tail_wgrad_reduce(const float* __restrict__ slab, int nslab, int Bn, float* __restrict__ dW, float* __restrict__ db) {
  const int n = tail_slab_floats(Bn);
  const int i = blockIdx.x * 32 + (threadIdx.x & 31);
  const float sum = slab_sum_fixed_order(slab + i, i < n ? nslab : 0, n);
  if (threadIdx.x >= 32 || i >= n) return;
  if (i < Bn * 32) { if (dW) dW[i] += sum; }
  else if (db) db[i - Bn * 32] += sum;
}

}
```

Baseline: 60680 frame-pairs/s.

## Decouple WaveNet activation row pitch from logical length across kernels

Adds separate row-pitch parameters (pL, pO, pV, dyP, etc.) to every WaveNet encoder and tail kernel so activations can be stored in padded or shared buffers whose row stride differs from the valid sequence length. The likely intent is aligned rows, or all layers sharing one allocation without per-layer reshaping, which avoids unaligned or bank-conflicting accesses and extra allocation or copies. It adds extra integer arguments and index arithmetic, and padding could waste memory bandwidth if the pitch is larger than needed.

```diff
diff --git a/audio-visual-vad_amd/csrc/wavenet.hip b/audio-visual-vad_amd/csrc/wavenet.hip
--- a/audio-visual-vad_amd/csrc/wavenet.hip
+++ b/audio-visual-vad_amd/csrc/wavenet.hip
@@ -7,55 +7,57 @@
 static inline int grid1(long n) { long b = (n + 255) / 256; return (int)(b > 8192 ? 8192 : (b < 1 ? 1 : b)); }
 
 __global__ void conv1d_fwd_generic(const float* __restrict__ x, const float* __restrict__ w, const float* __restrict__ bias,
-                                   const float* __restrict__ res, float* __restrict__ y, int B, int Cin, int Cout, int Lin,
-                                   int Lout, int fw, int dil, int relu_in, int res_off, int res_L) {
+                                   const float* __restrict__ res, float* __restrict__ y, int B, int Cin, int Cout, int xP,
+                                   int Lout, int yP, int fw, int dil, int relu_in, int res_off, int resP) {
   const long n = (long)B * Cout * Lout;
   for (long i = (long)blockIdx.x * blockDim.x + threadIdx.x; i < n; i += (long)gridDim.x * blockDim.x) {
     const int t = (int)(i % Lout);
     const int co = (int)((i / Lout) % Cout);
     const int b = (int)(i / ((long)Lout * Cout));
     float acc = bias ? bias[co] : 0.f;
-    const float* xb = x + (long)b * Cin * Lin + t;
+    const float* xb = x + (long)b * Cin * xP + t;
     const float* wr = w + (long)co * Cin * fw;
     for (int ci = 0; ci < Cin; ++ci)
       for (int k = 0; k < fw; ++k) {
-        float v = xb[(long)ci * Lin + k * dil];
+        float v = xb[(long)ci * xP + k * dil];
         if (relu_in) v = fmaxf(v, 0.f);
         acc = fmaf(wr[ci * fw + k], v, acc);
       }
-    if (res) acc += res[((long)b * Cout + co) * res_L + t + res_off];
-    y[i] = acc;
+    if (res) acc += res[((long)b * Cout + co) * resP + t + res_off];
+    y[((long)b * Cout + co) * yP + t] = acc;
   }
 }
 
 __global__ void conv1d_bwd_data_generic(const float* __restrict__ dy, const float* __restrict__ w,
                                         const float* __restrict__ xmask, const float* __restrict__ res, float* __restrict__ dx,
-                                        int B, int Cin, int Cout, int Lin, int Lout, int fw, int dil, int res_off, int res_L) {
+                                        int B, int Cin, int Cout, int Lin, int dxP, int Lout, int dyP, int fw, int dil, int res_off,
+                                        int res_L, int resP) {
   const long n = (long)B * Cin * Lin;
   for (long i = (long)blockIdx.x * blockDim.x + threadIdx.x; i < n; i += (long)gridDim.x * blockDim.x) {
     const int ti = (int)(i % Lin);
     const int ci = (int)((i / Lin) % Cin);
     const int b = (int)(i / ((long)Lin * Cin));
     float acc = 0.f;
-    if (!xmask || xmask[i] > 0.f) {
+    const long io = ((long)b * Cin + ci) * dxP + ti;
+    if (!xmask || xmask[io] > 0.f) {
       for (int k = 0; k < fw; ++k) {
         const int to = ti - k * dil;
         if (to < 0 || to >= Lout) continue;
-        const float* dyb = dy + (long)b * Cout * Lout + to;
-        for (int co = 0; co < Cout; ++co) acc = fmaf(w[((long)co * Cin + ci) * fw + k], dyb[(long)co * Lout], acc);
+        const float* dyb = dy + (long)b * Cout * dyP + to;
+        for (int co = 0; co < Cout; ++co) acc = fmaf(w[((long)co * Cin + ci) * fw + k], dyb[(long)co * dyP], acc);
       }
     }
-    if (res && ti >= res_off && ti - res_off < res_L) acc += res[((long)b * Cin + ci) * res_L + ti - res_off];
-    dx[i] = acc;
-  }
-}
-
-__global__ void __launch_bounds__(256) chan_sum_acc(const float* __restrict__ dy, float* __restrict__ db, int B, int C, int L) {
+    if (res && ti >= res_off && ti - res_off < res_L) acc += res[((long)b * Cin + ci) * resP + ti - res_off];
+    dx[io] = acc;
+  }
+}
+
+__global__ void __launch_bounds__(256) chan_sum_acc(const float* __restrict__ dy, float* __restrict__ db, int B, int C, int L, int P) {
   __shared__ float sm[256];
   const int c = blockIdx.x;
   float s = 0.f;
   for (int b = blockIdx.y; b < B; b += gridDim.y) {
-    const float* p = dy + ((long)b * C + c) * L;
+    const float* p = dy + ((long)b * C + c) * P;
     for (int t = threadIdx.x; t < L; t += 256) s += p[t];
   }
   sm[threadIdx.x] = s;
@@ -69,12 +71,12 @@
 
 __global__ void __launch_bounds__(256)
     narrow_conv1d_grads(const float* __restrict__ dy, const float* __restrict__ x, float* __restrict__ part,
-                        int B, int Cout, int Cin, int Lout, int Lin, int fw) {
+                        int B, int Cout, int Cin, int Lout, int dyP, int Lin, int fw) {
   __shared__ float sm[5][256];
   const int co = blockIdx.x, nw = Cin * fw;
   float acc[5] = {0.f, 0.f, 0.f, 0.f, 0.f};
   for (int b = blockIdx.y; b < B; b += gridDim.y) {
-    const float* p = dy + ((long)b * Cout + co) * Lout;
+    const float* p = dy + ((long)b * Cout + co) * dyP;
     const float* xb = x + (long)b * Cin * Lin;
     for (int t = threadIdx.x; t < Lout; t += 256) {
       const float g = p[t];
@@ -110,7 +112,7 @@
 __global__ void __launch_bounds__(256)
     wn_block_fwd_mfma(const float* __restrict__ s_in, const float* __restrict__ w_dil, const float* __restrict__ b_dil,
                       const float* __restrict__ w_dense, const float* __restrict__ b_dense, float* __restrict__ s_out,
-                      float* __restrict__ z_out, int B, int Lin, int dil) {
+                      float* __restrict__ z_out, int B, int Lin, int dil, int pL, int pO) {
   static_assert(MODE == 0 || MODE == 2, "s_out only, or z only");
   const int lane = threadIdx.x & 63;
   const int li = lane & 31, lh = lane >> 5;
@@ -136,13 +138,13 @@
   auto issue = [&](long tile) {
     const TilePos p = tile_pos(tile < ntiles ? tile : ntiles - 1, tiles_per_seq, li, Lo);
     const int b = p.b, tcl = p.ok ? p.t : 0;
-    const float* xp = s_in + (long)b * 32 * Lin + tcl + lh * dil;
-#pragma unroll
-    for (int c = 0; c < 32; ++c) xn[c] = xp[(long)c * Lin];
+    const float* xp = s_in + (long)b * 32 * pL + tcl + lh * dil;
+#pragma unroll
+    for (int c = 0; c < 32; ++c) xn[c] = xp[(long)c * pL];
     if (MODE == 0) {
-      const float* rp = s_in + (long)b * 32 * Lin + tcl + dil;
-#pragma unroll
-      for (int r = 0; r < 16; ++r) rn[r] = rp[(long)mfma32_row(r, lh) * Lin];
+      const float* rp = s_in + (long)b * 32 * pL + tcl + dil;
+#pragma unroll
+      for (int r = 0; r < 16; ++r) rn[r] = rp[(long)mfma32_row(r, lh) * pL];
     }
   };
   if (wave0 < ntiles) issue(wave0);
@@ -162,10 +164,10 @@
 #pragma unroll
     for (int s = 0; s < 32; ++s) acc = mfma32(wd[s], relu1(x[s]), acc);
     if (MODE == 2) {
-      float* zp = z_out + (long)b * 32 * Lo + t;
+      float* zp = z_out + (long)b * 32 * pO + t;
 #pragma unroll
       for (int r = 0; r < 16; ++r)
-        if (ok) zp[(long)mfma32_row(r, lh) * Lo] = acc[r];
+        if (ok) zp[(long)mfma32_row(r, lh) * pO] = acc[r];
     }
     if (MODE == 0) {
       f32x16 acc2;
@@ -173,10 +175,10 @@
       for (int r = 0; r < 16; ++r) acc2[r] = bsl[mfma32_row(r, lh)] + rv[r];
 #pragma unroll
       for (int r = 0; r < 16; ++r) acc2 = mfma32(we[r], relu1(acc[r]), acc2);
-      float* op = s_out + (long)b * 32 * Lo + t;
+      float* op = s_out + (long)b * 32 * pO + t;
 #pragma unroll
       for (int r = 0; r < 16; ++r)
-        if (ok) op[(long)mfma32_row(r, lh) * Lo] = acc2[r];
+        if (ok) op[(long)mfma32_row(r, lh) * pO] = acc2[r];
     }
   }
 }
@@ -186,7 +188,7 @@
 __device__ __forceinline__ void wn_block_fwd_body(float* wl, const float* __restrict__ s_in, const float* __restrict__ w_dil,
                                                   const float* __restrict__ b_dil, const float* __restrict__ w_dense,
                                                   const float* __restrict__ b_dense, float* __restrict__ s_out, int B, int Lin,
-                                                  int dil) {
+                                                  int dil, int pL, int pO) {
   const int lane = threadIdx.x & 63;
   const int li = lane & 31, lh = lane >> 5;
   const int Lo = Lin - dil;
@@ -196,12 +198,12 @@
   const float* wel = wl + WIMG_DENSE + li * WIMG_DENSE_PITCH + 4 * lh;
   const float* bzl = wl + WIMG_BDIL + 4 * lh;
   const float* bsl = wl + WIMG_BDENSE + 4 * lh;
-  const int rowL = Lin * 4, rowO = Lo * 4;
+  const int rowL = pL * 4, rowO = pO * 4;
   float wd[32], we[16];
 
   auto issue = [&](int tile, FwdTile& n) __attribute__((always_inline)) {
     const TilePos p = tile_pos(RESIDENT && tile >= ntiles ? ntiles - 1 : tile, tiles_per_seq, li, Lo);
-    const __amdgpu_buffer_rsrc_t rx = brsrc(s_in + (long)p.b * 32 * Lin, 32 * rowL);
+    const __amdgpu_buffer_rsrc_t rx = brsrc(s_in + (long)p.b * 32 * pL, 32 * rowL);
     const int offx = p.ok ? (p.t + lh * dil) * 4 : BUF_OOB;
 #pragma unroll
     for (int c = 0; c < 32; ++c) n.x[c] = bload(rx, offx, c * rowL);
@@ -222,7 +224,7 @@
     for (int r = 0; r < 16; ++r) acc2[r] = bsl[mfma32_row(r, 0)] + c.r[r];
 #pragma unroll
     for (int r = 0; r < 16; ++r) acc2 = mfma32(RESIDENT ? we[r] : wel[mfma32_row(r, 0)], relu1(acc[r]), acc2);
-    const __amdgpu_buffer_rsrc_t ro = brsrc(s_out + (long)p.b * 32 * Lo, 32 * rowO);
+    const __amdgpu_buffer_rsrc_t ro = brsrc(s_out + (long)p.b * 32 * pO, 32 * rowO);
 #pragma unroll
     for (int r = 0; r < 16; ++r) bstore(acc2[r], ro, offo, mfma32_row(r, 0) * rowO);
   };
@@ -245,23 +247,23 @@
 __global__ void __launch_bounds__(256)
     wn_block_fwd_buf(const float* __restrict__ s_in, const float* __restrict__ w_dil, const float* __restrict__ b_dil,
                      const float* __restrict__ w_dense, const float* __restrict__ b_dense, float* __restrict__ s_out, int B,
-                     int Lin, int dil) {
+                     int Lin, int dil, int pL, int pO) {
   __shared__ float wl[WIMG_SIZE];
-  wn_block_fwd_body<true>(wl, s_in, w_dil, b_dil, w_dense, b_dense, s_out, B, Lin, dil);
+  wn_block_fwd_body<true>(wl, s_in, w_dil, b_dil, w_dense, b_dense, s_out, B, Lin, dil, pL, pO);
 }
 
 __global__ void __launch_bounds__(256, 4)
     wn_block_fwd_occ(const float* __restrict__ s_in, const float* __restrict__ w_dil, const float* __restrict__ b_dil,
                      const float* __restrict__ w_dense, const float* __restrict__ b_dense, float* __restrict__ s_out, int B,
-                     int Lin, int dil) {
+                     int Lin, int dil, int pL, int pO) {
   __shared__ float wl[WIMG_SIZE];
-  wn_block_fwd_body<false>(wl, s_in, w_dil, b_dil, w_dense, b_dense, s_out, B, Lin, dil);
+  wn_block_fwd_body<false>(wl, s_in, w_dil, b_dil, w_dense, b_dense, s_out, B, Lin, dil, pL, pO);
 }
 
 __global__ void __launch_bounds__(512, 4)
     wn_block_fwd_dma(const float* __restrict__ s_in, const float* __restrict__ w_dil, const float* __restrict__ b_dil,
                      const float* __restrict__ w_dense, const float* __restrict__ b_dense, float* __restrict__ s_out, int B, int Lin,
-                     int dil) {
+                     int dil, int pL, int pO) {
   const int lane = threadIdx.x & 63, wave = threadIdx.x >> 6;
   const int li = lane & 31, lh = lane >> 5;
   const int Lo = Lin - dil;
@@ -275,7 +277,7 @@
   const float* wel = wts + WIMG_DENSE + li * WIMG_DENSE_PITCH + 4 * lh;
   const float* bzl = wts + WIMG_BDIL + 4 * lh;
   const float* bsl = wts + WIMG_BDENSE + 4 * lh;
-  const int rowL = Lin * 4, rowO = Lo * 4;
+  const int rowL = pL * 4, rowO = pO * 4;
   float* const tb = wl + __builtin_amdgcn_readfirstlane(wave) * 2048;
   const float* const xs = tb + lh * 1024 + li;
   const float* const rs = tb + 1024 + 4 * lh * 32 + li;
@@ -284,7 +286,7 @@
   for (int tile = w.first; tile < w.last; tile += w.stride) {
     const TilePos p = tile_pos(tile, tiles_per_seq, li, Lo);
     const int b = p.b, t0 = p.t0;
-    const __amdgpu_buffer_rsrc_t rx = brsrc(s_in + (long)b * 32 * Lin, 32 * rowL);
+    const __amdgpu_buffer_rsrc_t rx = brsrc(s_in + (long)b * 32 * pL, 32 * rowL);
 #pragma unroll
     for (int q = 0; q < 4; ++q)
       __builtin_amdgcn_raw_ptr_buffer_load_lds(rx, (__attribute__((address_space(3))) void*)(tb + q * 256), 16, dvo + t0 * 4,
@@ -319,7 +321,7 @@
     __builtin_amdgcn_sched_barrier(0);
 #pragma unroll
     for (int r = 0; r < 16; ++r) acc2 = mfma32(we16[r], relu1(acc[r]), acc2);
-    const __amdgpu_buffer_rsrc_t ro = brsrc(s_out + (long)b * 32 * Lo, 32 * rowO);
+    const __amdgpu_buffer_rsrc_t ro = brsrc(s_out + (long)b * 32 * pO, 32 * rowO);
 #pragma unroll
     for (int r = 0; r < 16; ++r) bstore(acc2[r], ro, offo, mfma32_row(r, 0) * rowO);
     __builtin_amdgcn_sched_barrier(0);
@@ -329,7 +331,7 @@
 __global__ void __launch_bounds__(256, 2)
     wn_block_fwd_w4(const float* __restrict__ s_in, const float* __restrict__ w_dil, const float* __restrict__ b_dil,
                     const float* __restrict__ w_dense, const float* __restrict__ b_dense, float* __restrict__ s_out, int B,
-                    int Lin, int dil) {
+                    int Lin, int dil, int pL, int pO) {
   const int lane = threadIdx.x & 63;
   const int li = lane & 31, lh = lane >> 5;
   const int Lo = Lin - dil;
@@ -342,14 +344,14 @@
   const float* wel = wl + WIMG_DENSE + li * WIMG_DENSE_PITCH + 4 * lh;
   const float* bzl = wl + WIMG_BDIL + 4 * lh;
   const float* bsl = wl + WIMG_BDENSE + 4 * lh;
-  const int rowL = Lin * 4, rowO = Lo * 4;
+  const int rowL = pL * 4, rowO = pO * 4;
 
   const TileWalkI w = xcd_walk_i(ntiles);
   for (int tile = w.first; tile < w.last; tile += w.stride) {
     const TilePos p = tile_pos<128>(tile, tiles_per_seq, 4 * li, Lo);
     const int b = p.b, t0 = p.t0, t = p.t;
-    const __amdgpu_buffer_rsrc_t rx = brsrc(s_in + (long)b * 32 * Lin, 32 * rowL);
-    const __amdgpu_buffer_rsrc_t ro = brsrc(s_out + (long)b * 32 * Lo, 32 * rowO);
+    const __amdgpu_buffer_rsrc_t rx = brsrc(s_in + (long)b * 32 * pL, 32 * rowL);
+    const __amdgpu_buffer_rsrc_t ro = brsrc(s_out + (long)b * 32 * pO, 32 * rowO);
     const int offx = (t + lh * dil) * 4;
     f4v x[32];
 #pragma unroll
@@ -411,7 +413,7 @@
 
 __global__ void __launch_bounds__(256)
     wn_block_bwd_dz_mfma(const float* __restrict__ dS, const float* __restrict__ Z, const float* __restrict__ w_dense,
-                         float* __restrict__ DZ, int B, int Lo) {
+                         float* __restrict__ DZ, int B, int Lo, int pO) {
   const int lane = threadIdx.x & 63;
   const int li = lane & 31, lh = lane >> 5;
   const int tiles_per_seq = tiles_per_sequence<32>(Lo);
@@ -428,12 +430,12 @@
     const TilePos p = tile_pos(tile, tiles_per_seq, li, Lo);
     const int b = p.b, t = p.t;
     const bool ok = p.ok;
-    const long base = (long)b * 32 * Lo + (ok ? t : 0);
+    const long base = (long)b * 32 * pO + (ok ? t : 0);
     float g[16], z[16];
 #pragma unroll
-    for (int s = 0; s < 16; ++s) g[s] = dS[base + (long)(2 * s + lh) * Lo];
-#pragma unroll
-    for (int r = 0; r < 16; ++r) z[r] = Z[base + (long)mfma32_row(r, lh) * Lo];
+    for (int s = 0; s < 16; ++s) g[s] = dS[base + (long)(2 * s + lh) * pO];
+#pragma unroll
+    for (int r = 0; r < 16; ++r) z[r] = Z[base + (long)mfma32_row(r, lh) * pO];
 #pragma unroll
     for (int s = 0; s < 16; ++s) g[s] = ok ? g[s] : 0.f;
     f32x16 acc;
@@ -443,13 +445,13 @@
     for (int s = 0; s < 16; ++s) acc = mfma32(wt[s], g[s], acc);
 #pragma unroll
     for (int r = 0; r < 16; ++r)
-      if (ok) DZ[base + (long)mfma32_row(r, lh) * Lo] = z[r] > 0.f ? acc[r] : 0.f;
+      if (ok) DZ[base + (long)mfma32_row(r, lh) * pO] = z[r] > 0.f ? acc[r] : 0.f;
   }
 }
 
 __global__ void __launch_bounds__(256)
     wn_block_bwd_dx_mfma(const float* __restrict__ DZ, const float* __restrict__ s_in, const float* __restrict__ dS_out,
-                         const float* __restrict__ w_dil, float* __restrict__ dS_in, int B, int Lin, int dil) {
+                         const float* __restrict__ w_dil, float* __restrict__ dS_in, int B, int Lin, int dil, int pL, int pO) {
   const int lane = threadIdx.x & 63;
   const int li = lane & 31, lh = lane >> 5;
   const int Lo = Lin - dil;
@@ -468,14 +470,14 @@
     const bool ok = p.ok;
     const int to = t - lh * dil;
     const bool okz = ok && to >= 0 && to < Lo;
-    const float* zp = DZ + (long)b * 32 * Lo + (okz ? to : 0);
-#pragma unroll
-    for (int s = 0; s < 32; ++s) dzn[s] = zp[(long)s * Lo];
+    const float* zp = DZ + (long)b * 32 * pO + (okz ? to : 0);
+#pragma unroll
+    for (int s = 0; s < 32; ++s) dzn[s] = zp[(long)s * pO];
     const bool okr = ok && t >= dil;
-    const float* sp = s_in + (long)b * 32 * Lin + (ok ? t : 0);
-    const float* rp = dS_out + (long)b * 32 * Lo + (okr ? t - dil : 0);
-#pragma unroll
-    for (int r = 0; r < 16; ++r) { svn[r] = sp[(long)mfma32_row(r, lh) * Lin]; rvn[r] = rp[(long)mfma32_row(r, lh) * Lo]; }
+    const float* sp = s_in + (long)b * 32 * pL + (ok ? t : 0);
+    const float* rp = dS_out + (long)b * 32 * pO + (okr ? t - dil : 0);
+#pragma unroll
+    for (int r = 0; r < 16; ++r) { svn[r] = sp[(long)mfma32_row(r, lh) * pL]; rvn[r] = rp[(long)mfma32_row(r, lh) * pO]; }
   };
   const TileWalk tw = xcd_walk(ntiles);
   if (tw.first < tw.last) issue(tw.first);
@@ -497,10 +499,10 @@
     for (int r = 0; r < 16; ++r) acc[r] = 0.f;
 #pragma unroll
     for (int s = 0; s < 32; ++s) acc = mfma32(wt[s], dz[s], acc);
-    float* op = dS_in + (long)b * 32 * Lin + t;
+    float* op = dS_in + (long)b * 32 * pL + t;
 #pragma unroll
     for (int r = 0; r < 16; ++r)
-      if (ok) op[(long)mfma32_row(r, lh) * Lin] = (sv[r] > 0.f ? acc[r] : 0.f) + rv[r];
+      if (ok) op[(long)mfma32_row(r, lh) * pL] = (sv[r] > 0.f ? acc[r] : 0.f) + rv[r];
   }
 }
 
@@ -508,14 +510,14 @@
 template <bool RESIDENT>
 __device__ __forceinline__ void wn_block_bwd_dx_body(float* wl, const float* __restrict__ DZ, const float* __restrict__ s_in,
                                                      const float* __restrict__ dS_out, const float* __restrict__ w_dil,
-                                                     float* __restrict__ dS_in, int B, int Lin, int dil) {
+                                                     float* __restrict__ dS_in, int B, int Lin, int dil, int pL, int pO) {
   const int lane = threadIdx.x & 63;
   const int li = lane & 31, lh = lane >> 5;
   const int Lo = Lin - dil;
   const int tiles_per_seq = tiles_per_sequence<32>(Lin);
   const int ntiles = B * tiles_per_seq;
   const float* wtl = wl + li * 2 + lh;
-  const int rowL = Lin * 4, rowO = Lo * 4;
+  const int rowL = pL * 4, rowO = pO * 4;
   float wt[32];
   auto issue = [&](int tile, DxTile& n) __attribute__((always_inline)) {
     const TilePos p = tile_pos(RESIDENT && tile >= ntiles ? ntiles - 1 : tile, tiles_per_seq, li, Lin);
@@ -523,9 +525,9 @@
     const int to = t - lh * dil;
     const bool okz = p.ok && to >= 0 && to < Lo;
     const bool okr = p.ok && t >= dil;
-    const __amdgpu_buffer_rsrc_t rz = brsrc(DZ + (long)p.b * 32 * Lo, 32 * rowO);
-    const __amdgpu_buffer_rsrc_t rs = brsrc(s_in + (long)p.b * 32 * Lin, 32 * rowL);
-    const __amdgpu_buffer_rsrc_t rg = brsrc(dS_out + (long)p.b * 32 * Lo, 32 * rowO);
+    const __amdgpu_buffer_rsrc_t rz = brsrc(DZ + (long)p.b * 32 * pO, 32 * rowO);
+    const __amdgpu_buffer_rsrc_t rs = brsrc(s_in + (long)p.b * 32 * pL, 32 * rowL);
+    const __amdgpu_buffer_rsrc_t rg = brsrc(dS_out + (long)p.b * 32 * pO, 32 * rowO);
     const int offz = okz ? to * 4 : BUF_OOB;
     const int offs = p.ok ? t * 4 + 4 * lh * rowL : BUF_OOB;
     const int offg = okr ? (t - dil) * 4 + 4 * lh * rowO : BUF_OOB;
@@ -536,7 +538,7 @@
   };
   auto compute = [&](int tile, const DxTile& c) __attribute__((always_inline)) {
     const TilePos p = tile_pos(tile, tiles_per_seq, li, Lin);
-    const __amdgpu_buffer_rsrc_t ro = brsrc(dS_in + (long)p.b * 32 * Lin, 32 * rowL);
+    const __amdgpu_buffer_rsrc_t ro = brsrc(dS_in + (long)p.b * 32 * pL, 32 * rowL);
     const int offs = p.ok ? p.t * 4 + 4 * lh * rowL : BUF_OOB;
     f32x16 acc;
 #pragma unroll
@@ -562,16 +564,16 @@
 
 __global__ void __launch_bounds__(256)
     wn_block_bwd_dx_buf(const float* __restrict__ DZ, const float* __restrict__ s_in, const float* __restrict__ dS_out,
-                        const float* __restrict__ w_dil, float* __restrict__ dS_in, int B, int Lin, int dil) {
+                        const float* __restrict__ w_dil, float* __restrict__ dS_in, int B, int Lin, int dil, int pL, int pO) {
   __shared__ float wl[WIMG_DIL_SIZE];
-  wn_block_bwd_dx_body<true>(wl, DZ, s_in, dS_out, w_dil, dS_in, B, Lin, dil);
+  wn_block_bwd_dx_body<true>(wl, DZ, s_in, dS_out, w_dil, dS_in, B, Lin, dil, pL, pO);
 }
 
 __global__ void __launch_bounds__(256, 4)
     wn_block_bwd_dx_occ(const float* __restrict__ DZ, const float* __restrict__ s_in, const float* __restrict__ dS_out,
-                        const float* __restrict__ w_dil, float* __restrict__ dS_in, int B, int Lin, int dil) {
+                        const float* __restrict__ w_dil, float* __restrict__ dS_in, int B, int Lin, int dil, int pL, int pO) {
   __shared__ float wl[WIMG_DIL_SIZE];
-  wn_block_bwd_dx_body<false>(wl, DZ, s_in, dS_out, w_dil, dS_in, B, Lin, dil);
+  wn_block_bwd_dx_body<false>(wl, DZ, s_in, dS_out, w_dil, dS_in, B, Lin, dil, pL, pO);
 }
 
 constexpr int WG_SLAB = 3 * 1024 + 64;
@@ -579,7 +581,7 @@
 
 __global__ void __launch_bounds__(256)
     wn_block_wgrad_mfma(const float* __restrict__ dS, const float* __restrict__ Z, const float* __restrict__ DZ,
-                        const float* __restrict__ s_in, float* __restrict__ slab, int B, int Lin, int dil) {
+                        const float* __restrict__ s_in, float* __restrict__ slab, int B, int Lin, int dil, int pL, int pO) {
   __shared__ float tile[4][32 * 33];
   __shared__ float red[WG_SLAB];
   const int lane = threadIdx.x & 63, wave = threadIdx.x >> 6;
@@ -618,14 +620,14 @@
     const TilePos p = tile_pos(tl, tiles_per_seq, li, Lo);
     const int b = p.b, t = p.t;
     const bool ok = p.ok;
-    const long oo = (long)b * 32 * Lo + (ok ? t : 0);
-    const long oi = (long)b * 32 * Lin + (ok ? t : 0);
+    const long oo = (long)b * 32 * pO + (ok ? t : 0);
+    const long oi = (long)b * 32 * pL + (ok ? t : 0);
     float v0[16], v1[16], v2[16], v3[16], v4[16];
-    gl(DZ + oo, Lo, v0);
-    gl(s_in + oi, Lin, v1);
-    gl(s_in + oi + dil, Lin, v2);
-    gl(dS + oo, Lo, v3);
-    gl(Z + oo, Lo, v4);
+    gl(DZ + oo, pO, v0);
+    gl(s_in + oi, pL, v1);
+    gl(s_in + oi + dil, pL, v2);
+    gl(dS + oo, pO, v3);
+    gl(Z + oo, pO, v4);
     float fa[16], fb[16];
     xpose(v0, ok, false, fa);
 #pragma unroll
@@ -665,7 +667,7 @@
                                                            const float* __restrict__ dS, const float* __restrict__ w_dil,
                                                            const float* __restrict__ b_dil, const float* __restrict__ w_dense,
                                                            const float* __restrict__ s_in, float* __restrict__ DZ,
-                                                           float* __restrict__ slab, int B, int Lin, int dil) {
+                                                           float* __restrict__ slab, int B, int Lin, int dil, int pL, int pO) {
   const int lane = threadIdx.x & 63, wave = threadIdx.x >> 6;
   const int li = lane & 31, lh = lane >> 5;
   const int Lo = Lin - dil;
@@ -696,12 +698,12 @@
 #pragma unroll
   for (int r = 0; r < 16; ++r) { acc0[r] = 0.f; acc1[r] = 0.f; acc2[r] = 0.f; }
   float bs_dz = 0.f, bs_ds = 0.f;
-  const int rowL = Lin * 4, rowO = Lo * 4;
+  const int rowL = pL * 4, rowO = pO * 4;
 
   auto issue = [&](int tile, DzwTile& n) __attribute__((always_inline)) {
     const TilePos p = tile_pos(tile < ntiles ? tile : ntiles - 1, tiles_per_seq, li, Lo);
-    const __amdgpu_buffer_rsrc_t rg = brsrc(dS + (long)p.b * 32 * Lo, 32 * rowO);
-    const __amdgpu_buffer_rsrc_t rx = brsrc(s_in + (long)p.b * 32 * Lin, 32 * rowL);
+    const __amdgpu_buffer_rsrc_t rg = brsrc(dS + (long)p.b * 32 * pO, 32 * rowO);
+    const __amdgpu_buffer_rsrc_t rx = brsrc(s_in + (long)p.b * 32 * pL, 32 * rowL);
     const int offg = p.ok ? p.t * 4 + lh * rowO : BUF_OOB;
     const int offx = p.ok ? (p.t + lh * dil) * 4 : BUF_OOB;
 #pragma unroll
@@ -712,7 +714,7 @@
   auto compute = [&](int tidx, const DzwTile& c) __attribute__((always_inline)) {
     const TilePos p = tile_pos(tidx, tiles_per_seq, li, Lo);
     const int offo = p.ok ? p.t * 4 + 4 * lh * rowO : BUF_OOB;
-    const __amdgpu_buffer_rsrc_t rz = brsrc(DZ + (long)p.b * 32 * Lo, 32 * rowO);
+    const __amdgpu_buffer_rsrc_t rz = brsrc(DZ + (long)p.b * 32 * pO, 32 * rowO);
     float x[32];
 #pragma unroll
     for (int s = 0; s < 32; ++s) x[s] = relu1(c.x[s]);
@@ -795,22 +797,22 @@
 __global__ void __launch_bounds__(256)
     wn_block_bwd_dz_wgrad_mfma(const float* __restrict__ dS, const float* __restrict__ w_dil, const float* __restrict__ b_dil,
                                const float* __restrict__ w_dense, const float* __restrict__ s_in, float* __restrict__ DZ,
-                               float* __restrict__ slab, int B, int Lin, int dil) {
+                               float* __restrict__ slab, int B, int Lin, int dil, int pL, int pO) {
   __shared__ float tile[4 * 2 * 32 * 33];
   __shared__ float red[WG_SLAB];
   __shared__ float wl[WIMG_DIL_SIZE + 32];
-  wn_block_bwd_dz_wgrad_body<true>(tile, red, wl, nullptr, dS, w_dil, b_dil, w_dense, s_in, DZ, slab, B, Lin, dil);
+  wn_block_bwd_dz_wgrad_body<true>(tile, red, wl, nullptr, dS, w_dil, b_dil, w_dense, s_in, DZ, slab, B, Lin, dil, pL, pO);
 }
 
 __global__ void __launch_bounds__(256, 2)
     wn_block_bwd_dz_wgrad_occ(const float* __restrict__ dS, const float* __restrict__ w_dil, const float* __restrict__ b_dil,
                                const float* __restrict__ w_dense, const float* __restrict__ s_in, float* __restrict__ DZ,
-                               float* __restrict__ slab, int B, int Lin, int dil) {
+                               float* __restrict__ slab, int B, int Lin, int dil, int pL, int pO) {
   __shared__ float tile[4 * 2 * 32 * 33];
   __shared__ float red[WG_SLAB];
   __shared__ float wl[WIMG_DIL_SIZE + 32];
   __shared__ float wtl[WIMG_DENSE_SIZE];
-  wn_block_bwd_dz_wgrad_body<false>(tile, red, wl, wtl, dS, w_dil, b_dil, w_dense, s_in, DZ, slab, B, Lin, dil);
+  wn_block_bwd_dz_wgrad_body<false>(tile, red, wl, wtl, dS, w_dil, b_dil, w_dense, s_in, DZ, slab, B, Lin, dil, pL, pO);
 }
 
 typedef float f4u __attribute__((ext_vector_type(4), aligned(4)));
@@ -818,7 +820,7 @@
 __global__ void __launch_bounds__(256, 2)
     wn_block_bwd_dzw_t(const float* __restrict__ dS, const float* __restrict__ w_dil, const float* __restrict__ b_dil,
                        const float* __restrict__ w_dense, const float* __restrict__ s_in, float* __restrict__ DZ,
-                       float* __restrict__ slab, int B, int Lin, int dil) {
+                       float* __restrict__ slab, int B, int Lin, int dil, int pL, int pO) {
   __shared__ float red[WG_SLAB];
   __shared__ float wl[WIMG_BDENSE];
   const int lane = threadIdx.x & 63;
@@ -850,16 +852,16 @@
     const bool full = t0 + 32 <= Lo;
     float x[32], g[16];
     {
-      const float* xp = s_in + (long)b * 32 * Lin + tcl + lh * dil;
-#pragma unroll
-      for (int c = 0; c < 32; ++c) x[c] = xp[(long)c * Lin];
-      const float* gp = dS + (long)b * 32 * Lo + tcl;
-#pragma unroll
-      for (int q = 0; q < 16; ++q) g[q] = gp[(long)(2 * q + lh) * Lo];
+      const float* xp = s_in + (long)b * 32 * pL + tcl + lh * dil;
+#pragma unroll
+      for (int c = 0; c < 32; ++c) x[c] = xp[(long)c * pL];
+      const float* gp = dS + (long)b * 32 * pO + tcl;
+#pragma unroll
+      for (int q = 0; q < 16; ++q) g[q] = gp[(long)(2 * q + lh) * pO];
     }
     float gc[16], xc0[16], xc1[16];
-    const float* rowS = dS + ((long)b * 32 + li) * Lo + t0 + 4 * lh;
-    const float* rowX = s_in + ((long)b * 32 + li) * Lin + t0 + 4 * lh;
+    const float* rowS = dS + ((long)b * 32 + li) * pO + t0 + 4 * lh;
+    const float* rowX = s_in + ((long)b * 32 + li) * pL + t0 + 4 * lh;
     if (full) {
 #pragma unroll
       for (int q = 0; q < 4; ++q) {
@@ -896,7 +898,7 @@
     for (int s = 0; s < 16; ++s) dzT = mfma32(g[s], wtp[66 * s], dzT);
 #pragma unroll
     for (int r = 0; r < 16; ++r) dzT[r] = zT[r] > 0.f ? dzT[r] : 0.f;
-    float* rowZ = DZ + ((long)b * 32 + li) * Lo + t0 + 4 * lh;
+    float* rowZ = DZ + ((long)b * 32 + li) * pO + t0 + 4 * lh;
     if (full) {
 #pragma unroll
       for (int q = 0; q < 4; ++q) {
@@ -958,6 +960,7 @@
 struct Plan {
   int n;
   int L[66];
+  int P[66];
   size_t s[66];
   size_t z, dz, ga, gb, dzt;
   size_t zs[66];
@@ -973,16 +976,17 @@
   p->L[0] = d->L - (d->fw - 1);
   for (int i = 0; i < p->n; ++i) p->L[i + 1] = p->L[i] - d->dilations_h[i] * (d->fw - 1);
   if (p->L[p->n] < 1) return AVVAD_EINVAL;
+  for (int i = 0; i <= p->n; ++i) p->P[i] = (int)align_up((size_t)p->L[i], 32);
   size_t off = 0;
   auto take = [&](size_t n) { size_t o = off; off += align_up(n, 64); return o; };
   const size_t B = d->B;
   if (d->save_for_backward) {
-    for (int i = 0; i <= p->n; ++i) p->s[i] = take(B * d->R * p->L[i]);
-    const size_t big = B * (size_t)(d->R > d->D ? d->R : d->D) * p->L[0];
+    for (int i = 0; i <= p->n; ++i) p->s[i] = take(B * d->R * p->P[i]);
+    const size_t big = B * (size_t)(d->R > d->D ? d->R : d->D) * p->P[0];
     p->z = take(big); p->dz = take(big); p->ga = take(big); p->gb = take(big);
-    p->dzt = take(B * d->Bn * p->L[p->n]);
+    p->dzt = take(B * d->Bn * p->P[p->n]);
     {
-      const size_t zb = (d->R == 32 && d->D == 32 && d->fw == 2 && p->n > 0) ? take(B * d->D * p->L[1]) : 0;
+      const size_t zb = (d->R == 32 && d->D == 32 && d->fw == 2 && p->n > 0) ? take(B * d->D * p->P[1]) : 0;
       for (int i = 0; i < p->n; ++i) p->zs[i] = zb;
     }
     {
@@ -993,9 +997,9 @@
     p->gslab = take(igemm::SLAB_FLOATS);
   } else {
     for (int i = 0; i < p->n; ++i) p->zs[i] = 0;
-    const size_t a = take(B * d->R * p->L[0]), b2 = take(B * d->R * p->L[0]);
+    const size_t a = take(B * d->R * p->P[0]), b2 = take(B * d->R * p->P[0]);
     for (int i = 0; i <= p->n; ++i) p->s[i] = (i & 1) ? b2 : a;
-    p->z = take(B * d->D * p->L[0]);
+    p->z = take(B * d->D * p->P[0]);
     p->dz = p->ga = p->gb = p->dzt = 0;
   }
   p->total = off;
@@ -1004,7 +1008,8 @@
 
 static inline bool mfma_shape(const avvad_wavenet_desc* d) { return d->R == 32 && d->D == 32 && d->fw == 2; }
 static inline bool buf_ok(int B, int Lin) {
-  return avvad_tune().wn_flat != 1 && (long)Lin * 32 * 4 + 4096 < (1L << 31) && (long)B * cdiv(Lin, 32) < (1L << 31);
+  return avvad_tune().wn_flat != 1 && (long)align_up((size_t)Lin, 32) * 32 * 4 + 4096 < (1L << 31) &&
+         (long)B * cdiv(Lin, 32) < (1L << 31);
 }
 
 enum class FwdForm { FLAT, BUF, OCC, WIDE, DMA };
@@ -1083,21 +1088,22 @@
 }
 
 static void launch_block_fwd(const float* s_in, const float* wd, const float* bd, const float* we, const float* be, float* s_out,
-                             int B, int Lin, int dil, hipStream_t s) {
+                             int B, int Lin, int dil, int pL, int pO, hipStream_t s) {
   const FwdChoice c = fwd_form(B, Lin, dil);
   const dim3 grid(c.grid);
   switch (c.form) {
-    case FwdForm::WIDE: hipLaunchKernelGGL(wn_block_fwd_w4, grid, dim3(256), 0, s, s_in, wd, bd, we, be, s_out, B, Lin, dil); break;
-    case FwdForm::DMA: hipLaunchKernelGGL(wn_block_fwd_dma, grid, dim3(512), 0, s, s_in, wd, bd, we, be, s_out, B, Lin, dil); break;
-    case FwdForm::OCC: hipLaunchKernelGGL(wn_block_fwd_occ, grid, dim3(256), 0, s, s_in, wd, bd, we, be, s_out, B, Lin, dil); break;
-    case FwdForm::BUF: hipLaunchKernelGGL(wn_block_fwd_buf, grid, dim3(256), 0, s, s_in, wd, bd, we, be, s_out, B, Lin, dil); break;
+    case FwdForm::WIDE: hipLaunchKernelGGL(wn_block_fwd_w4, grid, dim3(256), 0, s, s_in, wd, bd, we, be, s_out, B, Lin, dil, pL, pO); break;
+    case FwdForm::DMA: hipLaunchKernelGGL(wn_block_fwd_dma, grid, dim3(512), 0, s, s_in, wd, bd, we, be, s_out, B, Lin, dil, pL, pO); break;
+    case FwdForm::OCC: hipLaunchKernelGGL(wn_block_fwd_occ, grid, dim3(256), 0, s, s_in, wd, bd, we, be, s_out, B, Lin, dil, pL, pO); break;
+    case FwdForm::BUF: hipLaunchKernelGGL(wn_block_fwd_buf, grid, dim3(256), 0, s, s_in, wd, bd, we, be, s_out, B, Lin, dil, pL, pO); break;
     case FwdForm::FLAT:
-      hipLaunchKernelGGL(wn_block_fwd_mfma<0>, grid, dim3(256), 0, s, s_in, wd, bd, we, be, s_out, (float*)nullptr, B, Lin, dil);
+      hipLaunchKernelGGL(wn_block_fwd_mfma<0>, grid, dim3(256), 0, s, s_in, wd, bd, we, be, s_out, (float*)nullptr, B, Lin, dil, pL,
+                         pO);
       break;
   }
 }
 
-static int wgrad_conv1d(const float* dy, const float* x, float* dw, int B, int Cout, int Cin, int Lout, int Lin, int fw,
+static int wgrad_conv1d(const float* dy, const float* x, float* dw, int B, int Cout, int Cin, int Lout, int dyP, int xP, int fw,
                         int dil, int relu_in, hipStream_t s, float* slab) {
   const long K = (long)B * Lout;
   if (K > 0x7fffffffL) return AVVAD_EINVAL;
@@ -1105,29 +1111,29 @@
   int split = 1024 / (cdiv(Cout, 64) * cdiv(Cin * fw, 64));
   if (split > ktiles) split = ktiles;
   if (split < 1) split = 1;
-  igemm::RowSegK a{dy, Lout, (long)Cout * Lout, Cout, (int)K, Lout, 0, 0, 1, 0};
-  igemm::RowSegK b{x, Lin, (long)Cin * Lin, Cin * fw, (int)K, Lout, 0, relu_in, fw, dil};
+  igemm::RowSegK a{dy, dyP, (long)Cout * dyP, Cout, (int)K, Lout, 0, 0, 1, 0};
+  igemm::RowSegK b{x, xP, (long)Cin * xP, Cin * fw, (int)K, Lout, 0, relu_in, fw, dil};
   igemm::EpiStore e{dw, (long)Cin * fw, nullptr, 1};
   return igemm::launch<64, 64>(a, b, e, Cout, Cin * fw, (int)K, split, s, slab);
 }
 
-static void bias_grad(const float* dy, float* db, int B, int C, int L, hipStream_t s) {
+static void bias_grad(const float* dy, float* db, int B, int C, int L, int P, hipStream_t s) {
   if (!db) return;
-  hipLaunchKernelGGL(chan_sum_acc, dim3(C, 1), dim3(256), 0, s, dy, db, B, C, L);
-}
-
-static void launch_tail_fwd(const float* sN, const float* wb, const float* bb, float* out, int B, int R, int Bn, int Lv, int P,
-                            hipStream_t s) {
+  hipLaunchKernelGGL(chan_sum_acc, dim3(C, 1), dim3(256), 0, s, dy, db, B, C, L, P);
+}
+
+static void launch_tail_fwd(const float* sN, const float* wb, const float* bb, float* out, int B, int R, int Bn, int Lv, int pV,
+                            int P, hipStream_t s) {
   const TailFwdChoice c = tail_fwd_form(B, R, Bn, P);
   switch (c.form) {
-    case TailFwdForm::MFMA4: hipLaunchKernelGGL(tail_fwd_mfma<4>, dim3(c.grid), dim3(256), 0, s, sN, wb, bb, out, B, Bn, Lv, P); break;
-    case TailFwdForm::MFMA1: hipLaunchKernelGGL(tail_fwd_mfma<1>, dim3(c.grid), dim3(256), 0, s, sN, wb, bb, out, B, Bn, Lv, P); break;
-    case TailFwdForm::GENERIC: hipLaunchKernelGGL(tail_fwd_generic, dim3(P, B), dim3(256), 0, s, sN, wb, bb, out, R, Bn, Lv, P); break;
+    case TailFwdForm::MFMA4: hipLaunchKernelGGL(tail_fwd_mfma<4>, dim3(c.grid), dim3(256), 0, s, sN, wb, bb, out, B, Bn, Lv, pV, P); break;
+    case TailFwdForm::MFMA1: hipLaunchKernelGGL(tail_fwd_mfma<1>, dim3(c.grid), dim3(256), 0, s, sN, wb, bb, out, B, Bn, Lv, pV, P); break;
+    case TailFwdForm::GENERIC: hipLaunchKernelGGL(tail_fwd_generic, dim3(P, B), dim3(256), 0, s, sN, wb, bb, out, R, Bn, Lv, pV, P); break;
   }
 }
 
 static int launch_tail_bwd(const float* sN, const float* wb, const float* bb, const float* dout, float* dW, float* db, float* dS,
-                           float* dzt, float* slab, float* gslab, int B, int R, int Bn, int Lv, int P, hipStream_t s) {
+                           float* dzt, float* slab, float* gslab, int B, int R, int Bn, int Lv, int pV, int P, hipStream_t s) {
   const TailBwdChoice c = tail_bwd_form(B, Lv, R, Bn, P, dW || db);
   int rc;
   if (c.form == TailBwdForm::PAIR || c.form == TailBwdForm::FUSED) {
@@ -1135,20 +1141,20 @@
     const size_t lds = (size_t)tail_fused_lds_floats(Bn, pair ? 2 : 1) * sizeof(float);
     if ((rc = pair ? allow_large_lds<tail_bwd_wgrad_pair<8>>(lds, lds) : allow_large_lds<tail_bwd_wgrad_mfma<8>>(lds, lds))) return rc;
     hipLaunchKernelGGL(pair ? tail_bwd_wgrad_pair<8> : tail_bwd_wgrad_mfma<8>, dim3(c.grid), dim3(pair ? 512 : 256), lds, s, sN, wb,
-                       bb, dout, dS, slab, B, Lv, P);
+                       bb, dout, dS, slab, B, Lv, pV, P);
     hipLaunchKernelGGL(tail_wgrad_reduce, dim3(cdiv(tail_slab_floats(Bn), 32)), dim3(256), 0, s, slab, c.grid, Bn, dW, db);
     return AVVAD_OK;
   }
   if (c.form == TailBwdForm::MFMA)
     hipLaunchKernelGGL(tail_bwd_mfma, dim3(c.grid), dim3(256), (size_t)tail_wimg_floats(Bn) * sizeof(float), s, sN, wb, bb, dout,
-                       dzt, dS, B, Bn, Lv, P);
+                       dzt, dS, B, Bn, Lv, pV, P);
   else
-    hipLaunchKernelGGL(tail_bwd_dz_generic, dim3(grid1((long)B * Bn * Lv)), dim3(256), 0, s, sN, wb, bb, dout, dzt, B, R, Bn, Lv, P);
-  if (dW && (rc = wgrad_conv1d(dzt, sN, dW, B, Bn, R, Lv, Lv, 1, 1, 0, s, gslab))) return rc;
-  bias_grad(dzt, db, B, Bn, Lv, s);
+    hipLaunchKernelGGL(tail_bwd_dz_generic, dim3(grid1((long)B * Bn * Lv)), dim3(256), 0, s, sN, wb, bb, dout, dzt, B, R, Bn, Lv, pV, P);
+  if (dW && (rc = wgrad_conv1d(dzt, sN, dW, B, Bn, R, Lv, pV, pV, 1, 1, 0, s, gslab))) return rc;
+  bias_grad(dzt, db, B, Bn, Lv, pV, s);
   if (c.form == TailBwdForm::GENERIC)
     hipLaunchKernelGGL(conv1d_bwd_data_generic, dim3(grid1((long)B * R * Lv)), dim3(256), 0, s, dzt, wb, (const float*)nullptr,
-                       (const float*)nullptr, dS, B, R, Bn, Lv, Lv, 1, 1, 0, 0);
+                       (const float*)nullptr, dS, B, R, Bn, Lv, pV, Lv, pV, 1, 1, 0, 0, 0);
   return AVVAD_OK;
 }
 
@@ -1171,23 +1177,24 @@
   const int B = d->B, R = d->R, D = d->D, fw = d->fw;
   hipLaunchKernelGGL(conv1d_fwd_generic, dim3(grid1((long)B * R * p.L[0])), dim3(256), 0, s, wave, prm->causal_w,
                      d->use_bias ? prm->causal_b : (const float*)nullptr, (const float*)nullptr, ws + p.s[0], B, d->qc, R,
-                     d->L, p.L[0], fw, 1, 0, 0, 0);
+                     d->L, p.L[0], p.P[0], fw, 1, 0, 0, 0);
   for (int i = 0; i < p.n; ++i) {
     const int dil = d->dilations_h[i];
     const float* bd = d->use_bias ? prm->dil_b_h[i] : nullptr;
     const float* be = d->use_bias ? prm->dense_b_h[i] : nullptr;
     if (mfma_shape(d)) {
-      launch_block_fwd(ws + p.s[i], prm->dil_w_h[i], bd, prm->dense_w_h[i], be, ws + p.s[i + 1], B, p.L[i], dil, s);
+      launch_block_fwd(ws + p.s[i], prm->dil_w_h[i], bd, prm->dense_w_h[i], be, ws + p.s[i + 1], B, p.L[i], dil, p.P[i], p.P[i + 1], s);
     } else {
       float* z = ws + p.z;
       hipLaunchKernelGGL(conv1d_fwd_generic, dim3(grid1((long)B * D * p.L[i + 1])), dim3(256), 0, s, ws + p.s[i],
-                         prm->dil_w_h[i], bd, (const float*)nullptr, z, B, R, D, p.L[i], p.L[i + 1], fw, dil, 1, 0, 0);
+                         prm->dil_w_h[i], bd, (const float*)nullptr, z, B, R, D, p.P[i], p.L[i + 1], p.P[i + 1], fw, dil, 1, 0, 0);
       hipLaunchKernelGGL(conv1d_fwd_generic, dim3(grid1((long)B * R * p.L[i + 1])), dim3(256), 0, s, z, prm->dense_w_h[i], be,
-                         ws + p.s[i], ws + p.s[i + 1], B, D, R, p.L[i + 1], p.L[i + 1], 1, 1, 1, p.L[i] - p.L[i + 1], p.L[i]);
+                         ws + p.s[i], ws + p.s[i + 1], B, D, R, p.P[i + 1], p.L[i + 1], p.P[i + 1], 1, 1, 1, p.L[i] - p.L[i + 1],
+                         p.P[i]);
     }
   }
   launch_tail_fwd(ws + p.s[p.n], prm->bott_w, d->use_bias ? prm->bott_b : (const float*)nullptr, out, B, R, d->Bn, p.L[p.n],
-                  d->P, s);
+                  p.P[p.n], d->P, s);
   AVVAD_LAUNCH_CHECK();
   return AVVAD_OK;
 }
@@ -1196,7 +1203,7 @@
                                        const float* b_dense, float* s_out, int B, int Lin, int dil, avvad_stream_t sv) {
   AVVAD_ENTER();
   if (!s_in || !w_dil || !w_dense || !s_out || B <= 0 || dil < 1 || Lin - dil < 1) return AVVAD_EINVAL;
-  launch_block_fwd(s_in, w_dil, b_dil, w_dense, b_dense, s_out, B, Lin, dil, (hipStream_t)sv);
+  launch_block_fwd(s_in, w_dil, b_dil, w_dense, b_dense, s_out, B, Lin, dil, Lin, Lin - dil, (hipStream_t)sv);
   AVVAD_LAUNCH_CHECK();
   return AVVAD_OK;
 }
@@ -1218,7 +1225,7 @@
   float* GB = ws + p.gb;
   if ((rc = launch_tail_bwd(ws + p.s[p.n], prm->bott_w, d->use_bias ? prm->bott_b : (const float*)nullptr, dout, g->bott_w,
                             d->use_bias ? g->bott_b : (float*)nullptr, GA, ws + p.dzt, ws + p.slab, ws + p.gslab, B, R, Bn,
-                            p.L[p.n], d->P, s)))
+                            p.L[p.n], p.P[p.n], d->P, s)))
     return rc;
   WgradTab wtab;
   bool any_slab = false;
@@ -1236,60 +1243,60 @@
   for (int i = p.n - 1; i >= 0; --i) {
     float* const slab_i = ws + p.slab + (size_t)i * WG_MAXBLK * WG_SLAB;
     const int dil = d->dilations_h[i];
-    const int Li = p.L[i], Lo = p.L[i + 1];
+    const int Li = p.L[i], Lo = p.L[i + 1], pL = p.P[i], pO = p.P[i + 1];
     const float* si = ws + p.s[i];
     const float* bd = d->use_bias ? prm->dil_b_h[i] : nullptr;
     const bool fast = mfma_shape(d);
     float* Zi = fast ? ws + p.zs[i] : Z;
     if (!fast)
       hipLaunchKernelGGL(conv1d_fwd_generic, dim3(grid1((long)B * D * Lo)), dim3(256), 0, s, si, prm->dil_w_h[i], bd,
-                         (const float*)nullptr, Zi, B, R, D, Li, Lo, fw, dil, 1, 0, 0);
+                         (const float*)nullptr, Zi, B, R, D, pL, Lo, pO, fw, dil, 1, 0, 0);
     if (fast) {
       const bool any_grad = g->dil_w_h[i] || g->dense_w_h[i] || (d->use_bias && (g->dil_b_h[i] || g->dense_b_h[i]));
       const BwdChoice bc = bwd_form(B, Lo, d->shared_device != 0, any_grad);
       switch (bc.form) {
         case BwdForm::RESIDENT:
           hipLaunchKernelGGL(wn_block_bwd_dz_wgrad_mfma, dim3(bc.grid), dim3(256), 0, s, GA, prm->dil_w_h[i], bd,
-                             prm->dense_w_h[i], si, DZ, slab_i, B, Li, dil);
+                             prm->dense_w_h[i], si, DZ, slab_i, B, Li, dil, pL, pO);
           break;
         case BwdForm::OCC:
           hipLaunchKernelGGL(wn_block_bwd_dz_wgrad_occ, dim3(bc.grid), dim3(256), 0, s, GA, prm->dil_w_h[i], bd,
-                             prm->dense_w_h[i], si, DZ, slab_i, B, Li, dil);
+                             prm->dense_w_h[i], si, DZ, slab_i, B, Li, dil, pL, pO);
           break;
         case BwdForm::TRANSPOSED:
           hipLaunchKernelGGL(wn_block_bwd_dzw_t, dim3(bc.grid), dim3(256), 0, s, GA, prm->dil_w_h[i], bd, prm->dense_w_h[i], si,
-                             DZ, slab_i, B, Li, dil);
+                             DZ, slab_i, B, Li, dil, pL, pO);
           break;
         case BwdForm::UNFUSED:
           hipLaunchKernelGGL(wn_block_fwd_mfma<2>, dim3(bc.grid_z), dim3(256), 0, s, si, prm->dil_w_h[i], bd, prm->dense_w_h[i],
-                             (const float*)nullptr, (float*)nullptr, Zi, B, Li, dil);
-          hipLaunchKernelGGL(wn_block_bwd_dz_mfma, dim3(bc.grid_dz), dim3(256), 0, s, GA, Zi, prm->dense_w_h[i], DZ, B, Lo);
+                             (const float*)nullptr, (float*)nullptr, Zi, B, Li, dil, pL, pO);
+          hipLaunchKernelGGL(wn_block_bwd_dz_mfma, dim3(bc.grid_dz), dim3(256), 0, s, GA, Zi, prm->dense_w_h[i], DZ, B, Lo, pO);
           if (any_grad)
-            hipLaunchKernelGGL(wn_block_wgrad_mfma, dim3(bc.grid), dim3(256), 0, s, GA, Zi, DZ, si, slab_i, B, Li, dil);
+            hipLaunchKernelGGL(wn_block_wgrad_mfma, dim3(bc.grid), dim3(256), 0, s, GA, Zi, DZ, si, slab_i, B, Li, dil, pL, pO);
           break;
       }
       if (any_grad) note_slabs(i, slab_i, bc.grid);
       const DxChoice dc = dx_form(B, Li);
       switch (dc.form) {
         case DxForm::OCC:
-          hipLaunchKernelGGL(wn_block_bwd_dx_occ, dim3(dc.grid), dim3(256), 0, s, DZ, si, GA, prm->dil_w_h[i], GB, B, Li, dil);
+          hipLaunchKernelGGL(wn_block_bwd_dx_occ, dim3(dc.grid), dim3(256), 0, s, DZ, si, GA, prm->dil_w_h[i], GB, B, Li, dil, pL, pO);
           break;
         case DxForm::BUF:
-          hipLaunchKernelGGL(wn_block_bwd_dx_buf, dim3(dc.grid), dim3(256), 0, s, DZ, si, GA, prm->dil_w_h[i], GB, B, Li, dil);
+          hipLaunchKernelGGL(wn_block_bwd_dx_buf, dim3(dc.grid), dim3(256), 0, s, DZ, si, GA, prm->dil_w_h[i], GB, B, Li, dil, pL, pO);
           break;
         case DxForm::FLAT:
-          hipLaunchKernelGGL(wn_block_bwd_dx_mfma, dim3(dc.grid), dim3(256), 0, s, DZ, si, GA, prm->dil_w_h[i], GB, B, Li, dil);
+          hipLaunchKernelGGL(wn_block_bwd_dx_mfma, dim3(dc.grid), dim3(256), 0, s, DZ, si, GA, prm->dil_w_h[i], GB, B, Li, dil, pL, pO);
           break;
       }
     } else {
-      if (g->dense_w_h[i] && (rc = wgrad_conv1d(GA, Zi, g->dense_w_h[i], B, R, D, Lo, Lo, 1, 1, 1, s, ws + p.gslab))) return rc;
-      if (d->use_bias) bias_grad(GA, g->dense_b_h[i], B, R, Lo, s);
+      if (g->dense_w_h[i] && (rc = wgrad_conv1d(GA, Zi, g->dense_w_h[i], B, R, D, Lo, pO, pO, 1, 1, 1, s, ws + p.gslab))) return rc;
+      if (d->use_bias) bias_grad(GA, g->dense_b_h[i], B, R, Lo, pO, s);
       hipLaunchKernelGGL(conv1d_bwd_data_generic, dim3(grid1((long)B * D * Lo)), dim3(256), 0, s, GA, prm->dense_w_h[i], Zi,
-                         (const float*)nullptr, DZ, B, D, R, Lo, Lo, 1, 1, 0, 0);
-      if (g->dil_w_h[i] && (rc = wgrad_conv1d(DZ, si, g->dil_w_h[i], B, D, R, Lo, Li, fw, dil, 1, s, ws + p.gslab))) return rc;
-      if (d->use_bias) bias_grad(DZ, g->dil_b_h[i], B, D, Lo, s);
+                         (const float*)nullptr, DZ, B, D, R, Lo, pO, Lo, pO, 1, 1, 0, 0, 0);
+      if (g->dil_w_h[i] && (rc = wgrad_conv1d(DZ, si, g->dil_w_h[i], B, D, R, Lo, pO, pL, fw, dil, 1, s, ws + p.gslab))) return rc;
+      if (d->use_bias) bias_grad(DZ, g->dil_b_h[i], B, D, Lo, pO, s);
       hipLaunchKernelGGL(conv1d_bwd_data_generic, dim3(grid1((long)B * R * Li)), dim3(256), 0, s, DZ, prm->dil_w_h[i], si, GA,
-                         GB, B, R, D, Li, Lo, fw, dil, Li - Lo, Lo);
+                         GB, B, R, D, Li, pL, Lo, pO, fw, dil, Li - Lo, Lo, pO);
     }
     float* t = GA; GA = GB; GB = t;
   }
@@ -1299,17 +1306,17 @@
     {
       const int ny = B < 32 ? B : 32;
       float* part = ws + p.gslab;
-      hipLaunchKernelGGL(narrow_conv1d_grads, dim3(R, ny), dim3(256), 0, s, GA, wave, part, B, R, d->qc, p.L[0], d->L, fw);
+      hipLaunchKernelGGL(narrow_conv1d_grads, dim3(R, ny), dim3(256), 0, s, GA, wave, part, B, R, d->qc, p.L[0], p.P[0], d->L, fw);
       hipLaunchKernelGGL(narrow_conv1d_grads_sum, dim3(cdiv(R * 5, 256)), dim3(256), 0, s, part, ny, R, d->qc * fw, g->causal_w,
                          d->use_bias ? g->causal_b : (float*)nullptr);
     }
   } else {
-    if (g->causal_w && (rc = wgrad_conv1d(GA, wave, g->causal_w, B, R, d->qc, p.L[0], d->L, fw, 1, 0, s, ws + p.gslab))) return rc;
-    if (d->use_bias) bias_grad(GA, g->causal_b, B, R, p.L[0], s);
+    if (g->causal_w && (rc = wgrad_conv1d(GA, wave, g->causal_w, B, R, d->qc, p.L[0], p.P[0], d->L, fw, 1, 0, s, ws + p.gslab))) return rc;
+    if (d->use_bias) bias_grad(GA, g->causal_b, B, R, p.L[0], p.P[0], s);
   }
   if (dwave)
     hipLaunchKernelGGL(conv1d_bwd_data_generic, dim3(grid1((long)B * d->qc * d->L)), dim3(256), 0, s, GA, prm->causal_w,
-                       (const float*)nullptr, (const float*)nullptr, dwave, B, d->qc, R, d->L, p.L[0], fw, 1, 0, 0);
+                       (const float*)nullptr, (const float*)nullptr, dwave, B, d->qc, R, d->L, d->L, p.L[0], p.P[0], fw, 1, 0, 0, 0);
   AVVAD_LAUNCH_CHECK();
   return AVVAD_OK;
 }
diff --git a/audio-visual-vad_amd/csrc/wn_tail.h b/audio-visual-vad_amd/csrc/wn_tail.h
--- a/audio-visual-vad_amd/csrc/wn_tail.h
+++ b/audio-visual-vad_amd/csrc/wn_tail.h
@@ -92,18 +92,18 @@
 
 __global__ void __launch_bounds__(256)
     tail_fwd_generic(const float* __restrict__ s, const float* __restrict__ wb, const float* __restrict__ bb,
-                     float* __restrict__ out, int R, int Bn, int Lv, int P) {
+                     float* __restrict__ out, int R, int Bn, int Lv, int pV, int P) {
   const int b = blockIdx.y, p = blockIdx.x;
   int a, e;
   pool_bin(p, Lv, P, a, e);
-  const float* sb = s + (long)b * R * Lv;
+  const float* sb = s + (long)b * R * pV;
   for (int bn = threadIdx.x; bn < Bn; bn += 256) {
     const float* wr = wb + (long)bn * R;
     const float bias = bb ? bb[bn] : 0.f;
     float sum = 0.f;
     for (int t = a; t < e; ++t) {
       float z = bias;
-      for (int c = 0; c < R; ++c) z = fmaf(wr[c], sb[(long)c * Lv + t], z);
+      for (int c = 0; c < R; ++c) z = fmaf(wr[c], sb[(long)c * pV + t], z);
       sum += fmaxf(z, 0.f);
     }
     out[((long)b * Bn + bn) * P + p] = sum / (float)(e - a);
@@ -111,15 +111,16 @@
 }
 
 __global__ void tail_bwd_dz_generic(const float* __restrict__ s, const float* __restrict__ wb, const float* __restrict__ bb,
-                                    const float* __restrict__ dout, float* __restrict__ dz, int B, int R, int Bn, int Lv, int P) {
+                                    const float* __restrict__ dout, float* __restrict__ dz, int B, int R, int Bn, int Lv, int pV,
+                                    int P) {
   const long n = (long)B * Bn * Lv;
   for (long i = (long)blockIdx.x * blockDim.x + threadIdx.x; i < n; i += (long)gridDim.x * blockDim.x) {
     const int t = (int)(i % Lv);
     const int bn = (int)((i / Lv) % Bn);
     const int b = (int)(i / ((long)Lv * Bn));
     float z = bb ? bb[bn] : 0.f;
-    const float* sb = s + (long)b * R * Lv + t;
-    for (int c = 0; c < R; ++c) z = fmaf(wb[(long)bn * R + c], sb[(long)c * Lv], z);
+    const float* sb = s + (long)b * R * pV + t;
+    for (int c = 0; c < R; ++c) z = fmaf(wb[(long)bn * R + c], sb[(long)c * pV], z);
     float g = 0.f;
     if (z > 0.f) {
       const int p0 = (int)(((long)t * P) / Lv), p1 = (int)((((long)t + 1) * P + Lv - 1) / Lv);
@@ -129,14 +130,14 @@
         g += dout[((long)b * Bn + bn) * P + p] / (float)(e - a);
       }
     }
-    dz[i] = g;
+    dz[((long)b * Bn + bn) * pV + t] = g;
   }
 }
 
 template <int NT>
 __global__ void __launch_bounds__(256)
     tail_fwd_mfma(const float* __restrict__ s, const float* __restrict__ wb, const float* __restrict__ bb,
-                  float* __restrict__ out, int B, int Bn, int Lv, int P) {
+                  float* __restrict__ out, int B, int Bn, int Lv, int pV, int P) {
   const int lane = threadIdx.x & 63;
   const int li = lane & 31, lh = lane >> 5;
   const int ngrp = Bn / (32 * NT);
@@ -157,14 +158,14 @@
       bias[n] = bb ? bb[bn0 + n * 32 + li] : 0.f;
       sum[n] = 0.f;
     }
-    const float* sp = s + (long)b * 32 * Lv;
+    const float* sp = s + (long)b * 32 * pV;
     for (int t0 = a; t0 < e; t0 += 32) {
       const int t = t0 + li;
       const bool ok = t < e;
       const int tcl = ok ? t : a;
       float x[16];
 #pragma unroll
-      for (int k = 0; k < 16; ++k) x[k] = sp[(long)(2 * k + lh) * Lv + tcl];
+      for (int k = 0; k < 16; ++k) x[k] = sp[(long)(2 * k + lh) * pV + tcl];
 #pragma unroll
       for (int k = 0; k < 16; ++k) x[k] = ok ? x[k] : 0.f;
 #pragma unroll
@@ -188,7 +189,8 @@
 
 __global__ void __launch_bounds__(256)
     tail_bwd_mfma(const float* __restrict__ s, const float* __restrict__ wb, const float* __restrict__ bb,
-                  const float* __restrict__ dout, float* __restrict__ dzt, float* __restrict__ dS, int B, int Bn, int Lv, int P) {
+                  const float* __restrict__ dout, float* __restrict__ dzt, float* __restrict__ dS, int B, int Bn, int Lv, int pV,
+                  int P) {
   const int lane = threadIdx.x & 63;
   const int li = lane & 31, lh = lane >> 5;
   const int tiles_per_seq = (Lv + 31) >> 5;
@@ -201,10 +203,10 @@
     const int b = (int)(tile / tiles_per_seq);
     const int t = (int)(tile - (long)b * tiles_per_seq) * 32 + li;
     const bool ok = t < Lv;
-    const float* sp = s + (long)b * 32 * Lv + (ok ? t : 0);
+    const float* sp = s + (long)b * 32 * pV + (ok ? t : 0);
     float x[16];
 #pragma unroll
-    for (int k = 0; k < 16; ++k) x[k] = sp[(long)(2 * k + lh) * Lv];
+    for (int k = 0; k < 16; ++k) x[k] = sp[(long)(2 * k + lh) * pV];
 #pragma unroll
     for (int k = 0; k < 16; ++k) x[k] = ok ? x[k] : 0.f;
     const PoolWindow pw = pool_window(t, ok, Lv, P);
@@ -221,21 +223,22 @@
       }, dz);
 #pragma unroll
       for (int r = 0; r < 16; ++r)
-        if (ok) dzt[((long)b * Bn + nb + mfma32_row(r, lh)) * Lv + t] = dz[r];
+        if (ok) dzt[((long)b * Bn + nb + mfma32_row(r, lh)) * pV + t] = dz[r];
       float wt[16];
       tail_wt_frag(wl, nb, li, lh, wt);
       tail_ds_product(accS, wt, dz);
     }
 #pragma unroll
     for (int r = 0; r < 16; ++r)
-      if (ok) dS[((long)b * 32 + mfma32_row(r, lh)) * Lv + t] = accS[r];
+      if (ok) dS[((long)b * 32 + mfma32_row(r, lh)) * pV + t] = accS[r];
   }
 }
 
 template <int NBT, int WPT>
 __device__ __forceinline__ void tail_bwd_wgrad_body(const float* __restrict__ s, const float* __restrict__ wb,
                                                     const float* __restrict__ bb, const float* __restrict__ dout,
-                                                    float* __restrict__ dS, float* __restrict__ slab, int B, int Lv, int P) {
+                                                    float* __restrict__ dS, float* __restrict__ slab, int B, int Lv, int pV,
+                                                    int P) {
   static_assert((WPT == 1 || WPT == 2) && NBT % WPT == 0, "one wave per time tile, or two that halve the bottleneck rows");
   constexpr int Bn = NBT * 32, NH = NBT / WPT, NWAVES = 4 * WPT, NTHREADS = 64 * NWAVES, SLAB = tail_slab_floats(Bn);
   extern __shared__ float wl[];
@@ -253,14 +256,14 @@
   __syncthreads();
   f32x16 accW[NH] = {};
   float bsum[NH] = {};
-  const int rowV = Lv * 4;
+  const int rowV = pV * 4;
   const bool single = (Lv % P) == 0;
   auto one_tile = [&](long tile, bool live) __attribute__((always_inline)) {
     const int b = __builtin_amdgcn_readfirstlane((int)((live ? tile : 0) / tiles_per_seq));
     const int t = (int)((live ? tile : 0) - (long)b * tiles_per_seq) * 32 + li;
     const bool ok = live && t < Lv;
-    const __amdgpu_buffer_rsrc_t rs = brsrc(s + (long)b * 32 * Lv, 32 * rowV);
-    const __amdgpu_buffer_rsrc_t rd = brsrc(dS + (long)b * 32 * Lv, 32 * rowV);
+    const __amdgpu_buffer_rsrc_t rs = brsrc(s + (long)b * 32 * pV, 32 * rowV);
+    const __amdgpu_buffer_rsrc_t rd = brsrc(dS + (long)b * 32 * pV, 32 * rowV);
     const __amdgpu_buffer_rsrc_t rg = brsrc(dout + (long)b * Bn * P, Bn * P * 4);
     const int offs = ok ? t * 4 + lh * rowV : BUF_OOB;
     const int offd = ok ? t * 4 + 4 * lh * rowV : BUF_OOB;
@@ -353,15 +356,17 @@
 template <int NBT>
 __global__ void __launch_bounds__(256)
     tail_bwd_wgrad_mfma(const float* __restrict__ s, const float* __restrict__ wb, const float* __restrict__ bb,
-                        const float* __restrict__ dout, float* __restrict__ dS, float* __restrict__ slab, int B, int Lv, int P) {
-  tail_bwd_wgrad_body<NBT, 1>(s, wb, bb, dout, dS, slab, B, Lv, P);
+                        const float* __restrict__ dout, float* __restrict__ dS, float* __restrict__ slab, int B, int Lv, int pV,
+                        int P) {
+  tail_bwd_wgrad_body<NBT, 1>(s, wb, bb, dout, dS, slab, B, Lv, pV, P);
 }
 
 template <int NBT>
 __global__ void __launch_bounds__(512, 2)
     tail_bwd_wgrad_pair(const float* __restrict__ s, const float* __restrict__ wb, const float* __restrict__ bb,
-                        const float* __restrict__ dout, float* __restrict__ dS, float* __restrict__ slab, int B, int Lv, int P) {
-  tail_bwd_wgrad_body<NBT, 2>(s, wb, bb, dout, dS, slab, B, Lv, P);
+                        const float* __restrict__ dout, float* __restrict__ dS, float* __restrict__ slab, int B, int Lv, int pV,
+                        int P) {
+  tail_bwd_wgrad_body<NBT, 2>(s, wb, bb, dout, dS, slab, B, Lv, pV, P);
 }
 
 __global__ void __launch_bounds__(256)
```

Result: no change. 60860 frame-pairs/s (median of 6 runs) (+0.3%).
